# ZhendongWang6/Uformer

Hardware: AMD Instinct MI355X
Metric: restored images/sec (256x256, Uformer-B) (higher is better)
Workload: dtype bf16

## Files before the change

### include/uformer_hip.h

```cpp
#ifndef UFORMER_HIP_H
#define UFORMER_HIP_H

#include <stddef.h>
#include <stdint.h>

#ifdef __cplusplus
extern "C" {
#endif

#define UF_ABI_VERSION 1

typedef enum { UF_F32 = 0, UF_BF16 = 1, UF_F16 = 2 } uf_dtype;

#define UF_OK 0
#define UF_ERR_SHAPE (-1)
#define UF_ERR_UNSUPPORTED (-2)
#define UF_ERR_ALIGN (-3)
#define UF_ERR_LAUNCH (-4)
#define UF_ERR_WORKSPACE (-5)
#define UF_ERR_NULL (-6)

int uf_version(void);
int uf_last_error(char* buf, size_t n);

// ... 36 lines not shown

int uf_window_attention_fwd(const void* q, const void* k, const void* vt, const float* bias_dense,
                            const float* mask, int n_mask, void* out, int n_windows, int heads,
                            int head_dim, int H, int W, int shift, uf_dtype dtype, void* stream);

int uf_dwconv3x3_gelu_fwd(const void* x, const float* w9, const float* bias, void* out, int B,
                          int H, int W, int C, uf_dtype dtype, void* stream);
int uf_dwconv3x3_fwd(const void* x, const float* w9, const float* bias, void* out, int B, int H,
                     int W, int C, int gelu, uf_dtype dtype, void* stream);

int uf_dwconv3x3_pre_gelu_fwd(const void* x, const float* w9, const float* bias, void* pre_out, void* act_out, int B, int H,
                              int W, int C, uf_dtype dtype, void* stream);
int uf_dwconv3x3_gelu_in_pre_gelu_fwd(const void* pre_in, const float* w9, const float* bias, void* pre_out, void* act_out, int B, int H,
                                      int W, int C, uf_dtype dtype, void* stream);
int uf_dwconv3x3_mul_dgelu(const void* dy, const float* w9_flipped, const void* pre, void* out, int B, int H, int W, int C,
                           uf_dtype dtype, void* stream);

int uf_dwconv_linear2_fwd(const void* h1, const float* w9, const float* bdw, const void* W2_fm,
                          const float* b2, float* x, int ld, int B, int H, int W, int C,
                          uf_dtype dtype, void* stream);

typedef struct uf_block_params {
    const float* norm1_w;
    const float* norm1_b;
    const float* modulator;
    const float* rpb_dense;
    const float* rpb_fm;
    const float* rpb_tab;
    const void* wqkv_fm;
    const float* bqkv;
    const void* wproj;
    const void* wproj_fm;
    const float* bproj;
    const float* norm2_w;
    const float* norm2_b;
    const void* w1_fm;
    const float* b1;
    const float* wdw9;
    const float* bdw;
    const void* w2_fm;
    const float* b2;
    int32_t shift;
    int32_t heads;
    const float* qkv_dw9;
    const float* qkv_bdw;
} uf_block_params;

size_t uf_block_workspace_bytes(int M, int C, uf_dtype dtype);

int uf_lewin_attn_fwd(const uf_block_params* p, float* x, int ld, int B, int H, int W, int C,
                      const float* user_mask, int n_mask, uf_dtype dtype, void* ws,
                      size_t ws_bytes, void* stream);
int uf_leff_fwd(const uf_block_params* p, float* x, int ld, int B, int H, int W, int C,
                uf_dtype dtype, void* ws, size_t ws_bytes, void* stream);
int uf_ffn_fwd(float* x, int ld, const float* gamma, const float* beta, const void* W1_fm, const float* b1, const void* W2_fm,
               const float* b2, const float* scale, int B, int M, int C, uf_dtype dtype, void* stream);
int uf_mlp_fwd(const uf_block_params* p, float* x, int ld, int B, int H, int W, int C, uf_dtype dtype, void* ws, size_t ws_bytes,
               void* stream);
int uf_lewin_attn_train_fwd(const uf_block_params* p, const float* x, int ld, float* x1, int ld1, int B, int H, int W, int C,
                            const float* drop_attn, uf_dtype dtype, void* xn, void* q, void* k, void* vt, void* o, void* z, void* a1,
                            void* stream);
int uf_lewin_block_fwd(const uf_block_params* p, float* x, int ld, int B, int H, int W, int C,
                       const float* user_mask, int n_mask, uf_dtype dtype, void* ws,
                       size_t ws_bytes, void* stream);

int uf_lewin_block_train_fwd(const uf_block_params* p, float* x, int ld, int B, int H, int W, int C,
                             const float* drop_attn, const float* drop_leff, uf_dtype dtype, void* ws,
                             size_t ws_bytes, void* stream);

int uf_downsample_fwd(const float* x, int ld_x, const void* w, const float* bias, float* out,
                      int ld_o, int B, int H, int W, int C, uf_dtype dtype, void* stream);
int uf_downsample_fm_fwd(const float* x, int ld_x, const void* w, const void* w_fm, const float* bias, float* out,
                         int ld_o, int B, int H, int W, int C, uf_dtype dtype, void* stream);
int uf_upsample_fwd(const float* x, int ld_x, const void* w, const float* bias, float* out,
                    int ld_o, int B, int H, int W, int Cin, int Cout, uf_dtype dtype, void* stream);
int uf_input_proj_fwd(const float* img, const float* w27, const float* bias, float* out, int ld_o,
                      int B, int Cin, int H, int W, int E, void* stream);
int uf_output_proj_fwd(const float* x, int ld_x, const float* w, const float* bias,
                       const float* img, float* out, int B, int H, int W, int C2, int add_img,
                       void* stream);
int uf_output_proj_c_fwd(const float* x, int ld_x, const float* w, const float* bias,
                         const float* img, float* out, int B, int H, int W, int C2, int Cout, int add_img,
                         void* stream);

int uf_gelu_bwd(const void* a, const void* dy, void* dx, long long n, uf_dtype dtype, void* stream);
int uf_gelu_fwd(const void* a, void* y, long long n, uf_dtype dtype, void* stream);
int uf_linear_pre_gelu_fwd(const void* A, const void* W, const float* bias, void* out, void* act_out, int M, int N, int K,
                           uf_dtype dtype, void* stream);
int uf_linear_mul_dgelu(const void* A, const void* W, const float* bias, const void* pre, void* out, int M, int N, int K,
                        uf_dtype dtype, void* stream);
int uf_linear_residual_fwd(const void* A, const void* W, const float* bias, const float* resid, float* out, const float* scale,
                           int B, int H, int Wd, int N, int K, int windowed, int shift, uf_dtype dtype, void* stream);
size_t uf_layernorm_bwd_workspace_bytes(int rows, int C);
int uf_layernorm_bwd(const float* x, int ld_x, const float* gamma, const float* dy, int ld_dy, float* dx, int ld_dx,
                     float* dgamma, float* dbeta, int rows, int C, void* ws, size_t ws_bytes, void* stream);
int uf_layernorm_bwd_fused(const float* x, int ld_x, const float* gamma, const void* dy, int ld_dy, int dy_is_f32,
                           const float* add, float* dx, int ld_dx, float* dgamma, float* dbeta, int B, int H, int W, int C,
                           int windowed, int shift, uf_dtype dtype, void* ws, size_t ws_bytes, void* stream);
int uf_layernorm_bwd_cast(const float* x, int ld_x, const float* gamma, const void* dy, int ld_dy, int dy_is_f32,
                          const float* add, float* dx, int ld_dx, float* dgamma, float* dbeta, int B, int H, int W, int C,
                          int windowed, int shift, uf_dtype dtype, void* cast_out, const float* cast_scale, int cast_windowed, int cast_shift,
                          void* ws, size_t ws_bytes, void* stream);
size_t uf_linear_wgrad_workspace_bytes(int M, int N, int K);
int uf_linear_wgrad(const void* dY, int ldy, const void* X, int ldx, float* dW, float* db, int M, int N, int K,
                    uf_dtype dtype, void* ws, size_t ws_bytes, void* stream);
size_t uf_window_attention_bwd_workspace_bytes(int n_windows, int heads);
int uf_window_attention_bwd(const void* q, const void* k, const void* vt, const float* bias_dense, const float* mask,
                            int n_mask, const void* dO, int ldo, void* dq, void* dk, void* dvt, float* dbias,
                            int n_windows, int heads, int head_dim, int H, int W, int shift, uf_dtype dtype,
                            void* ws, size_t ws_bytes, void* stream);
int uf_window_attention_bwd_qkv(const void* q, const void* k, const void* vt, const float* bias_dense, const float* mask,
                                int n_mask, const void* dO, int ldo, void* dqkv, float* dbias, int n_windows, int heads,
                                int head_dim, int H, int W, int shift, uf_dtype dtype, void* ws, size_t ws_bytes, void* stream);
size_t uf_dwconv3x3_wgrad_workspace_bytes(int C, uf_dtype dtype);
int uf_dwconv3x3_wgrad(const void* h, const void* dc, float* dw9, float* dbias, int B, int H, int W, int C,
                       uf_dtype dtype, void* ws, size_t ws_bytes, void* stream);
size_t uf_dwconv3x3_bwd_workspace_bytes(int C, uf_dtype dtype);
int uf_dwconv3x3_bwd(const void* dc, const float* w9_flipped, const void* pre, void* da, float* dw9, float* dbias,
                     int B, int H, int W, int C, uf_dtype dtype, void* ws, size_t ws_bytes, void* stream);

size_t uf_rows_sum_workspace_bytes(int M, int N);
int uf_rows_sum(const void* X, int ld, float* out, int M, int N, uf_dtype dtype, void* ws, size_t ws_bytes, void* stream);
int uf_rpb_table_grad(const float* dbias_dense, float* dtable, int heads, void* stream);
int uf_im2col(const float* x, int ld_x, void* cols, int ldc, int B, int H, int W, int Cin, int k, int stride, int pad,
              int nchw, uf_dtype dtype, void* stream);
int uf_col2im(const void* dcols, int ldc, float* dx, int ld_dx, int B, int H, int W, int Cin, int k, int stride, int pad,
              int nchw, int accumulate, uf_dtype dtype, void* stream);

size_t uf_conv3x3_bwd_workspace_bytes(int B, int H, int W, int Cin, int Cout);
int uf_conv3x3_bwd(const float* x, int x_nchw, const float* dy, const float* act_out, float slope, const float* w, float* dx,
                   float* dW, float* db, int B, int H, int W, int Cin, int Cout, void* ws, size_t ws_bytes, void* stream);

int uf_residual_combine(const float* a, const void* b, int b_is_f32, float* out, const float* scale, int B, int H, int W,
                        int C, int windowed, int shift, uf_dtype dtype, void* stream);
int uf_grad_fork(const float* g1, const float* g2, float* sum_out, void* cast_out, const float* scale, int B, int H, int W,
                 int C, int windowed, int shift, uf_dtype dtype, void* stream);
int uf_qkv_grad_merge(const void* dq, const void* dk, const void* dvt, void* dqkv, int n_windows, int heads, int head_dim,
                      uf_dtype dtype, void* stream);

typedef struct uf_block_train_params {
    const float* norm1_w;  const float* norm1_b;  const float* norm2_w;  const float* norm2_b;
    const float* modulator;
    const float* rpb_dense;
    const void* wqkv;
    const void* wqkv_t;
    const float* bqkv;
    const void* wproj;  const void* wproj_t;  const float* bproj;
    const void* w1;     const void* w1_t;     const float* b1;
    const float* wdw9;  const float* wdw9_flip;  const float* bdw;
    const void* w2_t;
    int32_t shift, heads;
    const void* w2;
} uf_block_train_params;
typedef struct uf_block_grads {
    float* norm1_w;  float* norm1_b;  float* norm2_w;  float* norm2_b;
    float* modulator;
    float* rpb_table;
    float* wqkv;  float* bqkv;
    float* wproj; float* bproj;
    float* w1;    float* b1;
    float* wdw;   float* bdw;
    float* w2;    float* b2;
} uf_block_grads;
typedef struct uf_block_raw_params {
    const float* norm1_w;  const float* norm1_b;  const float* norm2_w;  const float* norm2_b;
    const float* modulator;
// ... 146 lines not shown
```

### uformer_amd/_lib.py

```python
from __future__ import annotations

import ctypes as C
import os
import threading

_HERE = os.path.dirname(os.path.abspath(__file__))
LIB_PATH = os.path.join(_HERE, "lib", "libuformer_hip.so")
LIB_PATH = os.environ.get("UFORMER_HIP_LIB", LIB_PATH)

UF_F32, UF_BF16, UF_F16 = 0, 1, 2

c_int, c_void_p, c_size_t, c_float_p = C.c_int, C.c_void_p, C.c_size_t, C.c_void_p


class BlockParams(C.Structure):
    _fields_ = [(n, C.c_void_p) for n in (
        "norm1_w", "norm1_b", "modulator", "rpb_dense", "rpb_fm", "rpb_tab", "wqkv_fm", "bqkv", "wproj", "wproj_fm", "bproj",
        "norm2_w", "norm2_b", "w1_fm", "b1", "wdw9", "bdw", "w2_fm", "b2")] + [
        ("shift", C.c_int32), ("heads", C.c_int32), ("qkv_dw9", C.c_void_p), ("qkv_bdw", C.c_void_p)]


class BlockTrainParams(C.Structure):
    _fields_ = [(n, C.c_void_p) for n in (
        "norm1_w", "norm1_b", "norm2_w", "norm2_b", "modulator", "rpb_dense", "wqkv", "wqkv_t", "bqkv", "wproj", "wproj_t", "bproj",
# ... 24 lines not shown
class ModelDesc(C.Structure):
    _fields_ = [
        ("embed_dim", C.c_int32), ("dd_in", C.c_int32), ("in_chans", C.c_int32),
        ("depths", C.c_int32 * 9),
        ("blocks", C.POINTER(BlockParams)),
        ("in_w27", C.c_void_p), ("in_b", C.c_void_p), ("out_w", C.c_void_p), ("out_b", C.c_void_p),
        ("down_w", C.c_void_p * 4), ("down_b", C.c_void_p * 4),
        ("up_w", C.c_void_p * 4), ("up_b", C.c_void_p * 4),
        ("down_w_fm", C.c_void_p * 4),
        ("cross", C.POINTER(CrossParams)),
    ]


class UnetDesc(C.Structure):
    _fields_ = [
        ("dim", C.c_int32),
        ("in_w27", C.c_void_p), ("in_b", C.c_void_p), ("c11_w1", C.c_void_p), ("c11_b1", C.c_void_p),
        ("w0", C.c_void_p * 9), ("b0", C.c_void_p * 9), ("w2", C.c_void_p * 9), ("b2", C.c_void_p * 9),
        ("w11", C.c_void_p * 9), ("b11", C.c_void_p * 9),
        ("pool_w", C.c_void_p * 4), ("pool_b", C.c_void_p * 4), ("up_w", C.c_void_p * 4), ("up_b", C.c_void_p * 4),
        ("out_w", C.c_void_p), ("out_b", C.c_void_p),
    ]


P = c_void_p
I = c_int
SIGNATURES = {
    "uf_version": (I, []),
    "uf_last_error": (I, [C.c_char_p, c_size_t]),
    "uf_timing_enable": (I, [I]),
    "uf_timing_report": (I, [C.c_char_p, c_size_t]),
    "uf_debug_set_tbuf": (I, [P]),
    "uf_weight_fm_elems": (c_size_t, [I, I]),
    "uf_pack_weight_fm": (I, [P, P, I, I, I, P]),
    "uf_window_partition": (I, [P, P, I, I, I, I, I, I, P]),
    "uf_window_reverse": (I, [P, P, I, I, I, I, I, I, P]),
    "uf_shift_mask": (I, [P, I, I, I, P]),
    "uf_layernorm_fwd": (I, [P, I, P, P, P, P, I, I, I, I, I, I, I, P]),
    "uf_linear_fwd": (I, [P, P, P, P, I, I, I, I, I, P]),
    "uf_qkv_fwd": (I, [P, P, P, P, P, P, I, I, I, I, P]),
    "uf_ln_qkv_fwd": (I, [P, I, P, P, P, P, P, P, P, P, I, I, I, I, I, I, I, P]),
    "uf_ln_convqkv_fwd": (I, [P, I, P, P, P, P, P, P, P, P, P, P, I, I, I, I, I, I, I, P]),
    "uf_ln_linear_gelu_fwd": (I, [P, I, P, P, P, P, P, I, I, I, I, P]),
    "uf_window_attention_fwd": (I, [P, P, P, P, P, I, P, I, I, I, I, I, I, I, P]),
    "uf_dwconv3x3_gelu_fwd": (I, [P, P, P, P, I, I, I, I, I, P]),
    "uf_dwconv3x3_fwd": (I, [P, P, P, P, I, I, I, I, I, I, P]),
    "uf_gelu_bwd": (I, [P, P, P, C.c_longlong, I, P]),
    "uf_gelu_fwd": (I, [P, P, C.c_longlong, I, P]),
    "uf_linear_pre_gelu_fwd": (I, [P, P, P, P, P, I, I, I, I, P]),
    "uf_linear_mul_dgelu": (I, [P, P, P, P, P, I, I, I, I, P]),
    "uf_dwconv3x3_pre_gelu_fwd": (I, [P, P, P, P, P, I, I, I, I, I, P]),
    "uf_dwconv3x3_gelu_in_pre_gelu_fwd": (I, [P, P, P, P, P, I, I, I, I, I, P]),
    "uf_dwconv3x3_mul_dgelu": (I, [P, P, P, P, I, I, I, I, I, P]),
    "uf_linear_residual_fwd": (I, [P, P, P, P, P, P, I, I, I, I, I, I, I, I, P]),
    "uf_layernorm_bwd_workspace_bytes": (c_size_t, [I, I]),
    "uf_layernorm_bwd": (I, [P, I, P, P, I, P, I, P, P, I, I, P, c_size_t, P]),
    "uf_layernorm_bwd_fused": (I, [P, I, P, P, I, I, P, P, I, P, P, I, I, I, I, I, I, I, P, c_size_t, P]),
    "uf_layernorm_bwd_cast": (I, [P, I, P, P, I, I, P, P, I, P, P, I, I, I, I, I, I, I, P, P, I, I, P, c_size_t, P]),
    "uf_linear_wgrad_workspace_bytes": (c_size_t, [I, I, I]),
    "uf_linear_wgrad": (I, [P, I, P, I, P, P, I, I, I, I, P, c_size_t, P]),
    "uf_window_attention_bwd_workspace_bytes": (c_size_t, [I, I]),
    "uf_window_attention_bwd": (I, [P, P, P, P, P, I, P, I, P, P, P, P, I, I, I, I, I, I, I, P, c_size_t, P]),
    "uf_window_attention_bwd_qkv": (I, [P, P, P, P, P, I, P, I, P, P, I, I, I, I, I, I, I, P, c_size_t, P]),
    "uf_dwconv3x3_wgrad_workspace_bytes": (c_size_t, [I, I]),
    "uf_dwconv3x3_wgrad": (I, [P, P, P, P, I, I, I, I, I, P, c_size_t, P]),
    "uf_dwconv3x3_bwd_workspace_bytes": (c_size_t, [I, I]),
    "uf_dwconv3x3_bwd": (I, [P, P, P, P, P, P, I, I, I, I, I, P, c_size_t, P]),
    "uf_dwconv_linear2_fwd": (I, [P, P, P, P, P, P, I, I, I, I, I, I, P]),
    "uf_block_workspace_bytes": (c_size_t, [I, I, I]),
    "uf_lewin_attn_fwd": (I, [C.POINTER(BlockParams), P, I, I, I, I, I, P, I, I, P, c_size_t, P]),
    "uf_leff_fwd": (I, [C.POINTER(BlockParams), P, I, I, I, I, I, I, P, c_size_t, P]),
    "uf_ffn_fwd": (I, [P, I, P, P, P, P, P, P, P, I, I, I, I, P]),
    "uf_cross_attn_fwd": (I, [C.POINTER(CrossParams), P, I, I, I, I, P]),
    "uf_mlp_fwd": (I, [C.POINTER(BlockParams), P, I, I, I, I, I, I, P, c_size_t, P]),
    "uf_lewin_attn_train_fwd": (I, [C.POINTER(BlockParams), P, I, P, I, I, I, I, I, P, I, P, P, P, P, P, P, P, P]),
    "uf_lewin_block_fwd": (I, [C.POINTER(BlockParams), P, I, I, I, I, I, P, I, I, P, c_size_t, P]),
    "uf_lewin_block_train_fwd": (I, [C.POINTER(BlockParams), P, I, I, I, I, I, P, P, I, P, c_size_t, P]),
    "uf_downsample_fwd": (I, [P, I, P, P, P, I, I, I, I, I, I, P]),
    "uf_downsample_fm_fwd": (I, [P, I, P, P, P, P, I, I, I, I, I, I, P]),
    "uf_upsample_fwd": (I, [P, I, P, P, P, I, I, I, I, I, I, I, P]),
    "uf_input_proj_fwd": (I, [P, P, P, P, I, I, I, I, I, I, P]),
    "uf_output_proj_fwd": (I, [P, I, P, P, P, P, I, I, I, I, I, P]),
    "uf_output_proj_c_fwd": (I, [P, I, P, P, P, P, I, I, I, I, I, I, P]),
    "uf_rows_sum_workspace_bytes": (c_size_t, [I, I]),
    "uf_rows_sum": (I, [P, I, P, I, I, I, P, c_size_t, P]),
    "uf_rpb_table_grad": (I, [P, P, I, P]),
    "uf_im2col": (I, [P, I, P, I, I, I, I, I, I, I, I, I, I, P]),
    "uf_col2im": (I, [P, I, P, I, I, I, I, I, I, I, I, I, I, I, P]),
    "uf_pack_block_train_bytes": (C.c_size_t, [I, I, I]),
    "uf_pack_block_train": (I, [P, I, I, I, I, P, C.c_size_t, P, P, P]),
    "uf_lewin_block_bwd_workspace_bytes": (C.c_size_t, [I, I, I, I, I, I]),
    "uf_lewin_block_bwd": (I, [P, P, P, P, P, P, P, I, I, I, I, I, P, C.c_size_t, P]),
    "uf_leff_bwd": (I, [P, P, P, P, P, P, I, I, I, I, I, P, C.c_size_t, P]),
    "uf_lewin_attn_bwd": (I, [P, P, P, P, P, P, I, I, I, I, I, P, C.c_size_t, P]),
    "uf_downsample_bwd_workspace_bytes": (C.c_size_t, [I, I, I, I, I, I]),
    "uf_downsample_bwd": (I, [P, I, P, P, P, I, I, P, P, I, I, I, I, I, I, P, C.c_size_t, P]),
    "uf_upsample_cat_bwd_workspace_bytes": (C.c_size_t, [I, I, I, I, I, I]),
    "uf_upsample_cat_bwd": (I, [P, I, P, I, P, P, P, P, I, I, I, I, I, I, P, C.c_size_t, P]),
    "uf_conv3x3_bwd_workspace_bytes": (C.c_size_t, [I, I, I, I, I]),
    "uf_conv3x3_bwd": (I, [P, I, P, P, C.c_float, P, P, P, P, I, I, I, I, I, P, C.c_size_t, P]),
    "uf_residual_combine": (I, [P, P, I, P, P, I, I, I, I, I, I, I, P]),
    "uf_grad_fork": (I, [P, P, P, P, P, I, I, I, I, I, I, I, P]),
    "uf_qkv_grad_merge": (I, [P, P, P, P, I, I, I, I, P]),
    "uf_charbonnier_workspace_bytes": (c_size_t, [C.c_longlong]),
    "uf_charbonnier_fwd_bwd": (I, [P, P, P, P, C.c_longlong, C.c_float, C.c_float, P, c_size_t, P]),
    "uf_adamw_step": (I, [P, P, P, P, P, I, C.c_double, C.c_double, C.c_double, C.c_double, C.c_double, I, C.c_double, P]),
    "uf_grad_scaler_check": (I, [P, P, I, P, P]),
    "uf_adamw_step_scaled": (I, [P, P, P, P, P, I, C.c_double, C.c_double, C.c_double, C.c_double, C.c_double, C.c_double, P, P]),
    "uf_grad_scaler_update": (I, [P, C.c_double, C.c_double, I, P]),
    "uf_image_metric_workspace_bytes": (c_size_t, [I, I, I, I]),
    "uf_batch_mse": (I, [P, P, P, I, I, I, I, I, P, c_size_t, P]),
    "uf_batch_ssim": (I, [P, P, P, I, I, I, I, P, c_size_t, P]),
    "uf_expand2square": (I, [P, P, P, I, I, I, I, I, P]),
    "uf_crop_clamp": (I, [P, P, I, I, I, I, I, I, P]),
    "uf_expand_canvas": (I, [P, P, P, I, I, I, I, I, I, P]),
    "uf_crop_clamp_canvas": (I, [P, P, I, I, I, I, I, I, I, P]),
    "uf_crop_augment": (I, [P, I, I, P, P, I, I, I, I, I, P]),
    "uf_crop_augment_c": (I, [P, I, I, P, P, I, I, I, I, I, I, P]),
    "uf_mixup": (I, [P, P, P, P, I, C.c_longlong, P]),
    "uf_uformer_workspace_bytes": (c_size_t, [C.POINTER(ModelDesc), I, I, I, I]),
    "uf_uformer_fwd": (I, [C.POINTER(ModelDesc), P, P, I, I, I, I, P, c_size_t, P]),
    "uf_window4_attention_fwd": (I, [P, I, P, P, I, I, I, I, I, I, I, P]),
    "uf_window4_attention_bwd": (I, [P, I, P, P, I, P, I, P, I, I, I, I, I, I, P]),
    "uf_rpb4_table_grad": (I, [P, P, I, I, P]),
    "uf_window4_partition": (I, [P, P, I, I, I, I, I, P]),
    "uf_window4_reverse": (I, [P, P, I, I, I, I, I, P]),
    "uf_lewin_block4_fwd": (I, [C.POINTER(Block4Params), P, I, I, I, I, I, P, P, I, P, c_size_t, P]),
    "uf_uformer_win4_workspace_bytes": (c_size_t, [C.POINTER(ModelDesc), I, I, I, I]),
    "uf_uformer_win4_fwd": (I, [C.POINTER(ModelDesc), C.POINTER(Block4Params), P, P, I, I, I, I, P, c_size_t, P]),
    "uf_conv_packed_elems": (c_size_t, [I, I, I]),
    "uf_conv3x3_fwd": (I, [P, I, P, P, P, I, P, I, I, I, I, I, I, I, I, I, P]),
    "uf_conv1x1_fwd": (I, [P, I, P, P, P, I, I, I, I, I, I, I, P]),
    "uf_conv4s2_fwd": (I, [P, I, P, P, P, I, I, I, I, I, I, I, P]),
    "uf_conv1x1_nchw_fwd": (I, [P, P, P, P, I, I, I, I, I, I, P]),
    "uf_unet_workspace_bytes": (c_size_t, [C.POINTER(UnetDesc), I, I, I, I]),
    "uf_unet_fwd": (I, [C.POINTER(UnetDesc), P, P, I, I, I, I, P, c_size_t, P]),
}

_lock = threading.Lock()
_lib = None


class UformerHipError(RuntimeError):
    pass


def load():
    global _lib
    if _lib is not None:
        return _lib
    with _lock:
        if _lib is not None:
            return _lib
        if not os.path.exists(LIB_PATH):
            raise UformerHipError(
                f"{LIB_PATH} not found: build it with `python __graft_entry__.py` "
                "(hipcc --offload-arch=gfx950).  There is no CPU / PyTorch fallback for the hot path.")
        lib = C.CDLL(LIB_PATH)
        older = os.environ.get("UF_ALLOW_OLDER_LIB") == "1"
        for name, (res, args) in SIGNATURES.items():
            if older and not hasattr(lib, name):
                continue
            fn = getattr(lib, name)
            fn.restype = res
            fn.argtypes = args
        if lib.uf_version() != 1:
# ... 15 lines not shown
```

### uformer_amd/csrc/uf_elementwise.hip

```cpp
#include "uf_internal.h"

namespace uf {
namespace {

template <bool REVERSE>
__global__ void window_copy_kernel(const u32x4* __restrict__ src, u32x4* __restrict__ dst, int rows, int chunks_per_row,
                                   int H, int W, int shift) {
    const long long idx = (long long)blockIdx.x * blockDim.x + threadIdx.x;
    if (idx >= (long long)rows * chunks_per_row) return;
    const int m = (int)(idx / chunks_per_row), c = (int)(idx - (long long)m * chunks_per_row);
    const int tok = window_row_to_token(m, H, W, shift);
    if (REVERSE) dst[(size_t)tok * chunks_per_row + c] = src[(size_t)m * chunks_per_row + c];
    else dst[(size_t)m * chunks_per_row + c] = src[(size_t)tok * chunks_per_row + c];
}

template <bool REVERSE, typename E>
__global__ void window_copy_elem_kernel(const E* __restrict__ src, E* __restrict__ dst, int rows, int C, int H, int W, int shift) {
    const long long idx = (long long)blockIdx.x * blockDim.x + threadIdx.x;
    if (idx >= (long long)rows * C) return;
    const int m = (int)(idx / C), c = (int)(idx - (long long)m * C);
    const int tok = window_row_to_token(m, H, W, shift);
    if (REVERSE) dst[(size_t)tok * C + c] = src[(size_t)m * C + c];
    else dst[(size_t)m * C + c] = src[(size_t)tok * C + c];
}

template <typename T, int C>
__global__ __launch_bounds__(256) void layernorm_kernel(const float* __restrict__ x, int ld_x, const float* __restrict__ gamma,
                                                        const float* __restrict__ beta, const float* __restrict__ modulator,
                                                        T* __restrict__ out, int rows, int H, int W, int windowed, int shift) {
    constexpr int LPR = (C / 4) < 64 ? (C / 4) : 64;
    constexpr int V4 = C / (4 * LPR);
    constexpr int RPB = 256 / LPR;
    const int sub = threadIdx.x % LPR;
    const int m = blockIdx.x * RPB + threadIdx.x / LPR;
    const bool live = m < rows;
    const int mc = live ? m : rows - 1;
    const int src = windowed ? window_row_to_token(mc, H, W, shift) : mc;
    f32x4 v[V4];
    float sum = 0.f;
#pragma unroll
    for (int i = 0; i < V4; ++i) {
        v[i] = *reinterpret_cast<const f32x4*>(x + (size_t)src * ld_x + (i * LPR + sub) * 4);
        sum += (v[i][0] + v[i][1]) + (v[i][2] + v[i][3]);
    }
    sum = allreduce<RedSum, LPR>(sum);
    const float mean = sum * (1.0f / C);
    float sq = 0.f;
#pragma unroll
    for (int i = 0; i < V4; ++i) {
        v[i] -= mean;
        sq += (v[i][0] * v[i][0] + v[i][1] * v[i][1]) + (v[i][2] * v[i][2] + v[i][3] * v[i][3]);
    }
    sq = allreduce<RedSum, LPR>(sq);
    const float rstd = 1.0f / sqrtf(sq * (1.0f / C) + 1e-5f);
    if (!live) return;
#pragma unroll
    for (int i = 0; i < V4; ++i) {
        const int c = (i * LPR + sub) * 4;
        const f32x4 g = *reinterpret_cast<const f32x4*>(gamma + c);
        const f32x4 b = *reinterpret_cast<const f32x4*>(beta + c);
        f32x4 y = v[i] * rstd * g + b;
        if (modulator) y += *reinterpret_cast<const f32x4*>(modulator + (size_t)(m & 63) * C + c);
        store4(out + (size_t)m * C + c, y);
    }
}

template <typename T> struct Vec16 {
    static_assert(sizeof(T) == 2, "2-byte operand type");
    static constexpr int N = 8;
    static __device__ __forceinline__ void load(const T* p, float* f) { unpack8<T>(*reinterpret_cast<const u32x4*>(p), f); }
    static __device__ __forceinline__ void store(T* p, const float* f) { *reinterpret_cast<u32x4*>(p) = pack8<T>(f); }
};
template <> struct Vec16<float> {
    static constexpr int N = 4;
    static __device__ __forceinline__ void load(const float* p, float* f) {
        const f32x4 r = *reinterpret_cast<const f32x4*>(p);
        f[0] = r[0]; f[1] = r[1]; f[2] = r[2]; f[3] = r[3];
    }
    static __device__ __forceinline__ void store(float* p, const float* f) {
        *reinterpret_cast<f32x4*>(p) = f32x4{f[0], f[1], f[2], f[3]};
    }
};

// ... 664 lines not shown
        }
#undef UF_IP2
        return check_launch("input_proj");
    }
    if (px == 8) hipLaunchKernelGGL(input_proj_kernel<8>, dim3((nx + 255) / 256, H, B), dim3(256), 0, (hipStream_t)stream, img, w27, bias, out, ld_o, B, Cin, H, W, E);
    else hipLaunchKernelGGL(input_proj_kernel<4>, dim3((nx + 255) / 256, H, B), dim3(256), 0, (hipStream_t)stream, img, w27, bias, out, ld_o, B, Cin, H, W, E);
    return check_launch("input_proj");
}

extern "C" int uf_output_proj_c_fwd(const float* x, int ld_x, const float* w, const float* bias, const float* img, float* out,
                                    int B, int H, int W, int C2, int Cout, int add_img, void* stream) {
    UF_REQUIRE(x && w && bias && out && (!add_img || img), UF_ERR_NULL, "uf_output_proj_fwd: null pointer");
    UF_REQUIRE(B > 0 && H > 0 && W > 0 && ld_x >= C2 && ld_x % 4 == 0, UF_ERR_SHAPE, "uf_output_proj_fwd: bad shape");
    UF_REQUIRE(Cout >= 1 && Cout <= 4, UF_ERR_UNSUPPORTED, "uf_output_proj_fwd: Cout=%d unsupported (1..4)", Cout);
    UF_REQUIRE((long long)B * H * W * ld_x < 0xffffffffLL && H / OP_R < 65535 && B <= 65535, UF_ERR_SHAPE, "uf_output_proj_fwd: tensor too large for 32-bit indexing");
    hipStream_t st = (hipStream_t)stream;
    const long long pix = (long long)B * H * W;
    ScopedTimer tm("output_proj", 18.0 * Cout * pix * C2, 4.0 * pix * (C2 + 2 * Cout), st);
#define UF_OP_CO(LAUNCH)                                                    \
    switch (Cout) {                                                         \
        case 1: LAUNCH(1) break;                                            \
        case 2: LAUNCH(2) break;                                            \
        case 3: LAUNCH(3) break;                                            \
        default: LAUNCH(4) break;                                           \
    }
    {
        const bool v1 = variant("head", 2) == 1;
        if (!v1 && (C2 == 16 || C2 == 32 || C2 == 64) && (long long)B * H * W * ld_x * 4 < 0xffffff00LL) {
            const int lpp = C2 / 4, tw = 2 * (256 / lpp), tiles_x = (W + tw - 1) / tw, tiles_y = (H + OP_R - 1) / OP_R;
            const int smem = (6 * (tw + 2) * C2 * 4 + 1023) / 1024 * 1024;
            const long long nt = (long long)tiles_x * tiles_y * B;
            if (nt < 0x7fffffffLL) {
#define UF_OP2(LPPV, COV)                                                                                                                             \
                {                                                                                                                                     \
                    auto kern = output_proj2_kernel<LPPV, COV>;                                                                                       \
                    static bool lds_done[64] = {};                                                                                                    \
                    if (int rc = ensure_dynamic_lds(reinterpret_cast<const void*>(kern), smem, lds_done, "output_proj")) return rc;                  \
                    hipLaunchKernelGGL(kern, dim3((unsigned)nt), dim3(256), smem, st, x, ld_x, w, bias, img, out, B, H, W, add_img, tiles_x, tiles_y); \
                }
#define UF_OP2_4(COV) UF_OP2(4, COV)
#define UF_OP2_8(COV) UF_OP2(8, COV)
#define UF_OP2_16(COV) UF_OP2(16, COV)
                if (lpp == 4) { UF_OP_CO(UF_OP2_4) } else if (lpp == 8) { UF_OP_CO(UF_OP2_8) } else { UF_OP_CO(UF_OP2_16) }
#undef UF_OP2_4
#undef UF_OP2_8
#undef UF_OP2_16
#undef UF_OP2
                return check_launch("output_proj");
            }
        }
    }
#define UF_OP1(LPPV, COV)                                                                                                               \
    {                                                                                                                                   \
        const unsigned nx = (unsigned)W * LPPV;                                                                                         \
        hipLaunchKernelGGL((output_proj_kernel<LPPV, COV>), dim3((nx + 255) / 256, (H + OP_R - 1) / OP_R, B), dim3(256), 0, st, x, ld_x, \
                           w, bias, img, out, B, H, W, add_img);                                                                        \
    }
#define UF_OP1_4(COV) UF_OP1(4, COV)
#define UF_OP1_8(COV) UF_OP1(8, COV)
#define UF_OP1_16(COV) UF_OP1(16, COV)
#define UF_OP1_32(COV) UF_OP1(32, COV)
    switch (C2) {
        case 16: UF_OP_CO(UF_OP1_4) break;
        case 32: UF_OP_CO(UF_OP1_8) break;
        case 64: UF_OP_CO(UF_OP1_16) break;
        case 128: UF_OP_CO(UF_OP1_32) break;
        default:
            set_error("uf_output_proj_fwd: C2=%d unsupported (16,32,64,128)", C2);
            return UF_ERR_UNSUPPORTED;
    }
#undef UF_OP1_4
#undef UF_OP1_8
#undef UF_OP1_16
#undef UF_OP1_32
#undef UF_OP1
#undef UF_OP_CO
    return check_launch("output_proj");
}

extern "C" int uf_output_proj_fwd(const float* x, int ld_x, const float* w, const float* bias, const float* img, float* out,
                                  int B, int H, int W, int C2, int add_img, void* stream) {
    return uf_output_proj_c_fwd(x, ld_x, w, bias, img, out, B, H, W, C2, 3, add_img, stream);
}
```

### uformer_amd/csrc/uf_internal.h

```cpp
#pragma once
#include "uf_common.h"

namespace uf {

enum ALoad { A_PLAIN = 0, A_FROM_R = 1, A_CONV_DOWN = 2 };
enum Epi {
    E_STORE_T = 0,
    E_STORE_T_GELU = 1,
    E_QKV = 2,
    E_RES_WINREV = 3,
    E_RES = 4,
    E_STORE_R = 5,
    E_UPSAMPLE = 6,
    E_STORE_T_PRE_GELU = 7,
    E_STORE_T_MUL_DGELU = 8
};

struct GemmParams {
    const void* A; int lda;
    const void* W;
    const void* W_fm = nullptr;
    const float* bias;
    int M, N, K;
    int H, W_, C;
    int shift;
    void* out; int ldo;
    const float* resid; int ldr;
    void* q; void* k; void* vt; int heads, hd; float qscale;
    int Cout;
    void* aux;
    const float* scale; int hw;
};

int launch_gemm(const GemmParams& p, int aload, int epi, uf_dtype dtype, hipStream_t stream);
int launch_down_dx(const void* dyT, int ld_dy, const void* w_pk_t, void* wc, float* dx, int ld_dx, int B, int H, int W, int Cin, int Cout, int accumulate, uf_dtype dtype,
                   hipStream_t st, bool* done);

constexpr int MAX_SIDE = 7, MAX_LANE_EVENTS = 8;
struct Lane { hipStream_t s[MAX_SIDE] = {}; hipEvent_t fork = nullptr, join[MAX_SIDE] = {}; int n = 0; hipEvent_t ev[MAX_LANE_EVENTS] = {}; int n_ev = 0; };
Lane* acquire_lane(int want, int* dev_out);
void release_lane(Lane* ln, int dev);
bool lane_events(Lane* ln, int want);

void debug_set_tbuf(void* p);
bool attn_block_supported(const uf_block_params* bp, const float* user_mask, uf_dtype dtype, int C, int heads);
int launch_attn_block(const uf_block_params* bp, float* x, int ld, int B, int H, int W, int C, uf_dtype dtype, void* h1_out, hipStream_t st,
                      const float* drop = nullptr, float* xo = nullptr, int ldo = 0);
int launch_leff2(const void* h1, const float* w9, const float* bdw, const void* W2, const float* b2, float* x, int ld, int B, int H, int W, int C,
                 uf_dtype dtype, const float* drop, hipStream_t st);

int launch_attn_block_train(const uf_block_params* bp, const float* x, int ld, float* x1, int ld1, int B, int H, int W, int C, uf_dtype dtype, const float* drop,
                            void* xn, void* q, void* k, void* vt, void* o, void* z, void* a1, hipStream_t st);

}
```

### uformer_amd/csrc/uf_leff2.hip

```cpp
#include <stdlib.h>

#include "uf_internal.h"
#include "uf_mconv.h"

namespace uf {
namespace {

struct Leff2Params {
    const void* h1;
    const float* w9; const float* bdw;
    const void* W2; const float* b2;
    float* x; int ld;
    const float* drop;
    int B, H, W;
    int n_tiles;
    unsigned long long* tbuf;
};

constexpr int KCW = 64;

template <typename T> __device__ __forceinline__ void cvt8(const char* p, float* f);
template <> __device__ __forceinline__ void cvt8<bf16>(const char* p, float* f) { unpack8<bf16>(*reinterpret_cast<const u32x4*>(p), f); }
template <> __device__ __forceinline__ void cvt8<f16>(const char* p, float* f) { unpack8<f16>(*reinterpret_cast<const u32x4*>(p), f); }
template <> __device__ __forceinline__ void cvt8<float>(const char* p, float* f) {
    const f32x4 a = *reinterpret_cast<const f32x4*>(p), b = *reinterpret_cast<const f32x4*>(p + 16);
    f[0] = a[0]; f[1] = a[1]; f[2] = a[2]; f[3] = a[3]; f[4] = b[0]; f[5] = b[1]; f[6] = b[2]; f[7] = b[3];
}
__device__ __forceinline__ void put8(bf16* p, const float* f) { *reinterpret_cast<u32x4*>(p) = pack8<bf16>(f); }
__device__ __forceinline__ void put8(f16* p, const float* f) { *reinterpret_cast<u32x4*>(p) = pack8<f16>(f); }
__device__ __forceinline__ void put8(float* p, const float* f) {
    *reinterpret_cast<f32x4*>(p) = f32x4{f[0], f[1], f[2], f[3]};
    *reinterpret_cast<f32x4*>(p + 4) = f32x4{f[4], f[5], f[6], f[7]};
}

template <typename T, int C, int NPG, int NC, int NBUF, int WPS, int PW = 4, int CP = 0>
__global__ __launch_bounds__((PW * NPG + NC) * 64, WPS) void leff2_kernel(const Leff2Params p) {
    constexpr int NP = PW * NPG;
    constexpr int MC = sizeof(T) == 2 ? 1 : 0;
    static_assert(PW == 4 || (PW == 8 && MC != 0), "8 producer waves per group: MFMA stencil only (two pixel tiles per wave)");
    static_assert(CP == 0 || (MC != 0 && PW == 4 && NPG == 1 && NC == 4 * CP), "consumer stencil jobs: MFMA stencil, 4 producers, one job per consumer wave");
    constexpr int PTW = 16 / PW - CP;
    constexpr int SR = 2;
    constexpr int SZ = sizeof(T);
    constexpr int TH = 8, TW = 8, BM = 64;
    constexpr int HID = 4 * C;
    constexpr int KC = KCW * NPG;
    constexpr int NIT = HID / KC;
    static_assert(HID % KC == 0, "interval width");
    constexpr int HW_ = TW + 2, HT = (TH + 2) * HW_;
    constexpr int PS = KCW * SZ;
    constexpr int CPP = PS / 16;
    constexpr int HGB = (HT * PS + 1023) / 1024 * 1024;
    constexpr int NHG = HGB / 1024;
    constexpr int TRB = KC * 4;
    constexpr int TGB = (10 * TRB + 1023) / 1024 * 1024;
    constexpr int NTI = TGB / 1024;
    constexpr int NHI = NPG * NHG;
    constexpr int NI = NHI + NTI;
    constexpr int NS = (NI + NP - 1) / NP;
    constexpr int BUFB = NPG * HGB + TGB;
    constexpr int SAT = KC * SZ + 16;
    constexpr int AT_BYTES = BM * SAT;
    constexpr int WN = (C / 16) < NC ? (C / 16) : NC, WM = NC / WN;
    static_assert(WM <= 4, "consumer grid");
    constexpr int TMW = 4 / WM, TNW = (C / 16) / WN;
    extern __shared__ __attribute__((aligned(16))) char smem[];
    char* Ring = smem;
    char* At0 = smem + NBUF * BUFB;

    const int tid = threadIdx.x, lane = tid & 63;
    const int wave = __builtin_amdgcn_readfirstlane(tid >> 6);
    const bool producer = wave < NP;
    const int fr = lane & 15, fg = lane >> 4;
    const int tiles_x = p.W / TW, tiles_y = p.H / TH;
    const int G = (int)gridDim.x;
    const int nk = (p.n_tiles - (int)blockIdx.x + G - 1) / G;
    const int NTOT = nk * NIT;
    const int bt = xcd_tile(blockIdx.x, p.n_tiles);
    auto tile_coords = [&](int k, int& b, int& y0, int& x0) {
        const int t = xcd_tile((int)blockIdx.x + k * G, p.n_tiles);
        b = t / (tiles_x * tiles_y);
        const int tr = t - b * (tiles_x * tiles_y);
        y0 = (tr / tiles_x) * TH; x0 = (tr % tiles_x) * TW;
    };
    const T* W2 = reinterpret_cast<const T*>(p.W2);

    const unsigned hshift = (fr & 1) * 16;
    unsigned msk[4];
#pragma unroll
    for (int d = 0; d < 4; ++d) msk[d] = ((fg & 1) == (fr >> 3) && d == ((fr & 7) >> 1)) ? 0xffffffffu : 0u;
    const int gq = (producer ? wave : wave - NP) & 3;
    int boff[5];
#pragma unroll
    for (int ks = 0; ks < 5; ++ks) {
        int tap = 2 * ks + (fg >> 1);
        tap = tap < 9 ? tap : 8;
        const int hy = (fr >> 3) + tap / 3, hx = (fr & 7) + tap % 3;
        boff[ks] = ((hy * HW_ + hx) * 8 + ((gq * 2 + (fg & 1)) ^ (hx & 6))) * 16;
    }
    Census census; census.begin();
    if (producer) {
        const unsigned lds0 = (unsigned)(uintptr_t)(__attribute__((address_space(3))) char*)smem;
        const unsigned lds_dummy = lds0 + NBUF * BUFB + 2 * AT_BYTES;
        u32x4 rsrc = {0u, 0u, (unsigned)__builtin_amdgcn_readfirstlane((int)((unsigned)(p.H * p.W) * (unsigned)(HID * SZ))), 0x00020000u};
        unsigned voff[NS];
        int issue_k = -1;
        auto set_issue_tile = [&](int k) {
            int b, y0, x0;
            tile_coords(k, b, y0, x0);
            const unsigned long long ia = (unsigned long long)(uintptr_t)(reinterpret_cast<const char*>(p.h1) + (size_t)b * p.H * p.W * HID * SZ);
            rsrc[0] = (unsigned)__builtin_amdgcn_readfirstlane((int)(unsigned)ia);
            rsrc[1] = (unsigned)__builtin_amdgcn_readfirstlane((int)(unsigned)(ia >> 32)) & 0xffffu;
#pragma unroll
            for (int s = 0; s < NS; ++s) {
                const int idx = wave + s * NP;
                voff[s] = 0xffffff00u;
                if (idx < NHI) {
                    const int g = idx / NHG, q = (idx - g * NHG) * 64 + lane;
                    const int hp = q / CPP, part = q - hp * CPP;
                    const int hy = hp / HW_, hx = hp - hy * HW_;
                    const int iy = y0 + hy - 1, ix = x0 + hx - 1;
                    const int piece = MC ? (part ^ (hx & 6)) : part;
                    if (hp < HT && iy >= 0 && iy < p.H && ix >= 0 && ix < p.W) voff[s] = ((unsigned)(iy * p.W + ix) * (unsigned)HID + (unsigned)(g * KCW)) * (unsigned)SZ + (unsigned)(piece * 16);
                }
            }
            issue_k = k;
        };
        auto issue = [&](int m) {
            const int k = m / NIT, it = m - k * NIT;
            if (k != issue_k) set_issue_tile(k);
            const unsigned slot = lds0 + (unsigned)(m % NBUF) * BUFB;
#pragma unroll
            for (int s = 0; s < NS; ++s) {
                const int idx = wave + s * NP;
                if (idx < NHI) {
                    dma_buffer_to_lds(rsrc, voff[s], (unsigned)(it * KC * SZ), slot + (unsigned)idx * 1024u);
                } else if (idx < NI) {
                    const int q = (idx - NHI) * 64 + lane;
                    int row = q / (KC / 4);
                    const int c4 = (q - row * (KC / 4)) * 4;
                    row = row > 9 ? 9 : row;
                    const float* src = (row < 9 ? p.w9 + (size_t)row * HID : p.bdw) + it * KC + c4;
                    dma_global_to_lds(src, slot + NPG * HGB + (unsigned)(idx - NHI) * 1024u);
                } else {
                    dma_buffer_to_lds(rsrc, 0xffffff00u, 0u, lds_dummy);
                }
            }
// ... 53 lines not shown
            t1 = __builtin_readcyclecounter(); tw += t1 - t0; t0 = t1;
            if (NBUF >= 3 && i + NBUF - 1 < NTOT) wait_dma<(NBUF - 2) * NS>(); else wait_dma<0>();
            lds_barrier();
            t1 = __builtin_readcyclecounter(); tbar += t1 - t0; t0 = t1;
        }
        if (p.tbuf && lane == 0 && (bt & 63) == 0) { p.tbuf[((bt >> 6) * 16 + wave) * 4] = tw; p.tbuf[((bt >> 6) * 16 + wave) * 4 + 1] = tbar; p.tbuf[((bt >> 6) * 16 + wave) * 4 + 2] = producer; }
        return;
    }

    const int cw = wave - NP;
    const int wm = cw / WN, wn = cw % WN;
    constexpr int WKS = (SZ == 4 && TNW >= 4) ? 1 : 2;
    Frag<T> wf[WKS][TNW];
    const __amdgpu_buffer_rsrc_t wrs = __builtin_amdgcn_make_buffer_rsrc(const_cast<T*>(W2), 0, C * HID * SZ, 0x00020000);
    const int wlane = lane * 8 * SZ;
    auto w2_load = [&](int sub, int ks, int slot) {
#pragma unroll
        for (int i = 0; i < TNW; ++i) {
            const int soff = (((wn * TNW + i) * (HID / 32) + sub * 2 + ks) * 64) * 8 * SZ;
            if constexpr (SZ == 2) {
                wf[slot][i].v = __builtin_bit_cast(u32x4, __builtin_amdgcn_raw_buffer_load_b128(wrs, wlane, soff, 0));
            } else {
                wf[slot][i].lo = __builtin_bit_cast(f32x4, __builtin_amdgcn_raw_buffer_load_b128(wrs, wlane, soff, 0));
                wf[slot][i].hi = __builtin_bit_cast(f32x4, __builtin_amdgcn_raw_buffer_load_b128(wrs, wlane + 16, soff, 0));
            }
        }
    };
    auto w2_issue = [&](int sub) {
        if constexpr (WKS == 2) { w2_load(sub, 0, 0); w2_load(sub, 1, 1); }
    };

    f32x4 acc[TNW][TMW];
#pragma unroll
    for (int i = 0; i < TNW; ++i)
#pragma unroll
        for (int j = 0; j < TMW; ++j) acc[i][j] = f32x4{0.f, 0.f, 0.f, 0.f};

    constexpr bool XPRE = SZ == 2 && TNW * TMW <= 4 && CP == 0;
    f32x4 xres[XPRE ? TNW : 1][XPRE ? TMW : 1];
    auto x_ptr = [&](int b, int y0, int x0, int i, int j) -> float* {
        const int n = (wn * TNW + i) * 16 + fg * 4;
        const int pm = (wm * TMW + j) * 16 + fr;
        return p.x + ((size_t)(b * p.H + y0 + (pm >> 3)) * p.W + x0 + (pm & 7)) * p.ld + n;
    };
    w2_issue(0);
    lds_barrier();
    unsigned long long ctw = 0, ctbar = 0, ct0 = __builtin_readcyclecounter(), ct1;
#pragma unroll 1
    for (int j = 0; j <= NTOT; ++j) {
        if (j >= 1) {
            const int m = j - 1, k = m / NIT, it = m - k * NIT;
            int tb = 0, ty0 = 0, tx0 = 0;
            if (it == NIT - 1) {
                tile_coords(k, tb, ty0, tx0);
                if constexpr (XPRE) {
#pragma unroll
                    for (int i = 0; i < TNW; ++i)
#pragma unroll
                        for (int jj = 0; jj < TMW; ++jj) xres[i][jj] = *reinterpret_cast<const f32x4*>(x_ptr(tb, ty0, tx0, i, jj));
                }
            }
            const char* At = At0 + (m & 1) * AT_BYTES;
#pragma unroll
            for (int g = 0; g < NPG; ++g) {
                const int sub = it * NPG + g;
#pragma unroll
                for (int ks = 0; ks < 2; ++ks) {
                    if constexpr (WKS == 1) w2_load(sub, ks, 0);
                    Frag<T> af[TMW];
#pragma unroll
                    for (int jj = 0; jj < TMW; ++jj)
                        load_frag(af[jj], reinterpret_cast<const T*>(At + ((wm * TMW + jj) * 16 + fr) * SAT + (g * KCW + ks * 32 + fg * 8) * SZ));
                    __builtin_amdgcn_sched_barrier(0);
#pragma unroll
                    for (int ii = 0; ii < TNW; ++ii)
#pragma unroll
                        for (int jj = 0; jj < TMW; ++jj) mma16(acc[ii][jj], wf[WKS == 2 ? ks : 0][ii], af[jj]);
                    __builtin_amdgcn_sched_barrier(0);
                }
                if (sub + 1 < NIT * NPG) w2_issue(sub + 1);
                else if (j < NTOT) w2_issue(0);
                __builtin_amdgcn_sched_barrier(0);
            }
            if (it == NIT - 1) {
                const float dscale = p.drop ? p.drop[tb] : 1.0f;
#pragma unroll
                for (int i = 0; i < TNW; ++i) {
                    const f32x4 b2 = *reinterpret_cast<const f32x4*>(p.b2 + (wn * TNW + i) * 16 + fg * 4);
#pragma unroll
                    for (int jj = 0; jj < TMW; ++jj) {
                        float* xp = x_ptr(tb, ty0, tx0, i, jj);
                        f32x4 r;
                        if constexpr (XPRE) r = xres[i][jj]; else r = *reinterpret_cast<const f32x4*>(xp);
                        *reinterpret_cast<f32x4*>(xp) = r + (acc[i][jj] + b2) * dscale;
                        acc[i][jj] = f32x4{0.f, 0.f, 0.f, 0.f};
                    }
                }
            }
        }
        if constexpr (CP > 0) {
            if (j < NTOT) {
                const char* Hs = Ring + (j % NBUF) * BUFB;
                const float* Wl = reinterpret_cast<const float*>(Ring + (j % NBUF) * BUFB + NPG * HGB);
                mconv_job<T, 1, KC, SAT, 2 * HW_ * PS>(Hs, Wl, At0 + (j & 1) * AT_BYTES, gq, 4 - CP + (cw >> 2), boff, msk, hshift, fr, fg);
            }
        }
        ct1 = __builtin_readcyclecounter(); ctw += ct1 - ct0; ct0 = ct1;
        lds_barrier();
        ct1 = __builtin_readcyclecounter(); ctbar += ct1 - ct0; ct0 = ct1;
    }
    if (p.tbuf && lane == 0 && (bt & 63) == 0) { p.tbuf[((bt >> 6) * 16 + wave) * 4] = ctw; p.tbuf[((bt >> 6) * 16 + wave) * 4 + 1] = ctbar; p.tbuf[((bt >> 6) * 16 + wave) * 4 + 2] = 0; }
    if (cw == 0 && lane == 0) {
        Census c2 = census;
        if (p.tbuf) { unsigned long long* o = p.tbuf + 65536 + (size_t)bt * 8; o[0] = c2.t0; o[1] = __builtin_readcyclecounter(); o[2] = c2.r0; o[3] = wall_clock64();
            o[4] = (unsigned long long)__builtin_amdgcn_s_getreg((31 << 11) | 4) | ((unsigned long long)__builtin_amdgcn_s_getreg((31 << 11) | 20) << 32); }
    }
}

template <typename T, int C, int NPG, int NC, int NBUF, int WPS, int PW = 4, int CP = 0>
int launch_v(const Leff2Params& p, hipStream_t st) {
    constexpr int SZ = sizeof(T), KC = KCW * NPG;
    constexpr int HGB = (100 * KCW * SZ + 1023) / 1024 * 1024, TGB = (10 * KC * 4 + 1023) / 1024 * 1024;
    constexpr int smem = NBUF * (NPG * HGB + TGB) + 2 * 64 * (KC * SZ + 16) + 1024;
    static_assert(smem <= 160 * 1024, "LDS budget");
    auto kern = leff2_kernel<T, C, NPG, NC, NBUF, WPS, PW, CP>;
    static bool lds_done[64] = {};
    if (int rc = ensure_dynamic_lds(reinterpret_cast<const void*>(kern), smem, lds_done, "leff2")) return rc;
    const long long M = (long long)p.B * p.H * p.W;
    char name[96] = "";
    if (timing_enabled()) snprintf(name, sizeof(name), "leff2_%s_c%d_np%d_nc%d %lldx%dx%d", TypeName<T>::s, C, PW * NPG, NC, M, C, 4 * C);
    {
        ScopedTimer tm(name, 2.0 * M * C * 4 * C + 18.0 * M * 4 * C, (double)M * 4 * C * SZ + (double)M * C * 8, st);
        const int pe = variant("persist", -1);
        const bool pays = C <= 32 || C >= 256 || (C == 128 && p.n_tiles <= 1024);
        const bool persist = pe >= 0 ? pe != 0 : pays;
        constexpr int waves = PW * NPG + NC;
        constexpr int by_lds = (160 * 1024) / smem, by_waves = 32 / waves, by_regs = (WPS * 4) / waves > 0 ? (WPS * 4) / waves : 1;
        constexpr int per_cu = by_lds < by_waves ? (by_lds < by_regs ? by_lds : by_regs) : (by_waves < by_regs ? by_waves : by_regs);
        const int resident = 256 * (per_cu < 1 ? 1 : per_cu);
        int grid = p.n_tiles;
        if (persist && p.n_tiles > resident) {
            const int rounds = (p.n_tiles + resident - 1) / resident;
            grid = ((p.n_tiles + rounds - 1) / rounds + 7) / 8 * 8;
        }
        hipLaunchKernelGGL(kern, dim3((unsigned)grid), dim3(waves * 64), smem, st, p);
    }
    return check_launch("leff2");
}

constexpr int NB512 = 3, NB256 = 3, NB256E = 3;
template <typename T, int C>
int launch_c(const Leff2Params& p, hipStream_t st) {
    const int tiles = p.B * (p.H / 8) * (p.W / 8);
    if constexpr (sizeof(T) == 2 && C >= 32) {
        const int ev = variant("leff2", 0);
        const bool force = ev == 1, never = ev == 2;
        if constexpr (C == 128) { if (!never && (force || tiles <= 1024)) return launch_v<T, C, 1, 4, 2, 6, 8>(p, st); }
        else if constexpr (C == 256) { if (!never && (force || tiles <= 256)) return launch_v<T, C, 1, 8, NB256E, 4, 8>(p, st); }
        else if constexpr (C == 512) { if (force) return launch_v<T, C, 1, 8, 4, 4, 8>(p, st); }
        else { if (force) return launch_v<T, C, 1, 4, 2, 6, 8>(p, st); }
    }
    if constexpr (sizeof(T) == 2) {
        if constexpr (C <= 128) return launch_v<T, C, 1, 4, 2, 6>(p, st);
        else if constexpr (C == 256) return launch_v<T, C, 1, 4, NB256, 4>(p, st);
        else return launch_v<T, C, 1, 8, NB512, 3>(p, st);
    } else {
        (void)tiles;
        if constexpr (C <= 256) return launch_v<T, C, 1, 4, 2, 2>(p, st);
        else return launch_v<T, C, 1, 4, 2, 2>(p, st);
    }
}

template <typename T>
int launch_t(const Leff2Params& p, int C, hipStream_t st) {
    switch (C) {
        case 16: return launch_c<T, 16>(p, st);
        case 32: return launch_c<T, 32>(p, st);
        case 64: return launch_c<T, 64>(p, st);
        case 128: return launch_c<T, 128>(p, st);
        case 256: return launch_c<T, 256>(p, st);
        case 512: return launch_c<T, 512>(p, st);
        default:
            set_error("leff2: C=%d unsupported (16,32,64,128,256,512)", C);
            return UF_ERR_UNSUPPORTED;
    }
}

}
unsigned long long* debug_get_tbuf();
}

using namespace uf;

namespace uf {
int launch_leff2(const void* h1, const float* w9, const float* bdw, const void* W2, const float* b2, float* x, int ld, int B, int H, int W, int C,
                 uf_dtype dtype, const float* drop, hipStream_t st) {
    UF_REQUIRE(h1 && w9 && bdw && W2 && b2 && x, UF_ERR_NULL, "uf_dwconv_linear2_fwd: null pointer");
    UF_REQUIRE(B > 0 && H >= 8 && W >= 8 && H % 8 == 0 && W % 8 == 0, UF_ERR_SHAPE, "uf_dwconv_linear2_fwd: B=%d H=%d W=%d (multiples of 8)", B, H, W);
    UF_REQUIRE(ld >= C && ld % 4 == 0, UF_ERR_ALIGN, "uf_dwconv_linear2_fwd: ld=%d", ld);
    UF_REQUIRE(((uintptr_t)h1 % 16) == 0 && ((uintptr_t)W2 % 16) == 0 && ((uintptr_t)x % 16) == 0 && ((uintptr_t)w9 % 16) == 0 &&
                   ((uintptr_t)bdw % 16) == 0 && ((uintptr_t)b2 % 16) == 0,
               UF_ERR_ALIGN, "uf_dwconv_linear2_fwd: operands must be 16-byte aligned");
    UF_REQUIRE((long long)H * W * 4LL * C * (long long)dtype_size(dtype) < 0xffffff00LL, UF_ERR_SHAPE,
               "uf_dwconv_linear2_fwd: one image of the hidden tensor must stay under 4 GiB (32-bit buffer offsets)");
    UF_REQUIRE((long long)B * H * W < 0x7fffffffLL / 4, UF_ERR_SHAPE, "uf_dwconv_linear2_fwd: too many tokens");
    Leff2Params p{};
    p.tbuf = debug_get_tbuf();
    p.h1 = h1; p.w9 = w9; p.bdw = bdw; p.W2 = W2; p.b2 = b2; p.x = x; p.ld = ld; p.B = B; p.H = H; p.W = W; p.drop = drop;
    p.n_tiles = B * (H / 8) * (W / 8);
    if (dtype == UF_BF16) return launch_t<bf16>(p, C, st);
    if (dtype == UF_F16) return launch_t<f16>(p, C, st);
    if (dtype == UF_F32) return launch_t<float>(p, C, st);
    set_error("uf_dwconv_linear2_fwd: dtype %d", (int)dtype);
    return UF_ERR_UNSUPPORTED;
}
}

extern "C" int uf_dwconv_linear2_fwd(const void* h1, const float* w9, const float* bdw, const void* W2, const float* b2,
                                     float* x, int ld, int B, int H, int W, int C, uf_dtype dtype, void* stream) {
    return uf::launch_leff2(h1, w9, bdw, W2, b2, x, ld, B, H, W, C, dtype, nullptr, (hipStream_t)stream);
}
```

### uformer_amd/csrc/uf_model.hip

```cpp
#include <stdlib.h>

#include <mutex>
#include <vector>

#include "uf_internal.h"

namespace uf {

int launch_layernorm(const float* x, int ld_x, const float* gamma, const float* beta, const float* modulator, void* out,
                     int rows, int H, int W, int C, int windowed, int shift, uf_dtype dtype, hipStream_t st);

int launch_unpack_weight_fm(const void* fm, void* w, int N, int K, uf_dtype dtype, hipStream_t st);

namespace {

struct BlockWs {
    char* a;
    char* h1;
    char* h2;
    char* wr;
};

bool wide_block(size_t C) { return C > 512; }

// ... 16 lines not shown
}

bool mlp_block(const uf_block_params* p) { return !p->wdw9 && !p->bdw; }

bool conv_block(const uf_block_params* p) { return p->qkv_dw9 && p->qkv_bdw; }

int check_block_args(const uf_block_params* p, const float* x, int ld, int B, int H, int W, int C, uf_dtype dtype) {
    UF_REQUIRE(p && x, UF_ERR_NULL, "block: null pointer");
    UF_REQUIRE(!p->qkv_dw9 == !p->qkv_bdw, UF_ERR_NULL, "block: qkv_dw9 and qkv_bdw must both be set (ConvProjection, token_projection = 'conv') or both be NULL");
    UF_REQUIRE(!(conv_block(p) && wide_block((size_t)C)), UF_ERR_UNSUPPORTED, "block: token_projection = 'conv' is built for C <= 512 (got C=%d)", C);
    UF_REQUIRE(!p->wdw9 == !p->bdw, UF_ERR_NULL, "block: wdw9 and bdw must both be set (LeFF) or both be NULL (Mlp, token_mlp = 'ffn')");
    UF_REQUIRE(!(mlp_block(p) && wide_block((size_t)C)), UF_ERR_UNSUPPORTED, "block: token_mlp = 'ffn' is built for C <= 512 (got C=%d)", C);
    UF_REQUIRE(dtype_ok(dtype), UF_ERR_UNSUPPORTED, "block: dtype %d", (int)dtype);
    UF_REQUIRE(B > 0 && H >= 8 && W >= 8 && H % 8 == 0 && W % 8 == 0, UF_ERR_SHAPE, "block: B=%d H=%d W=%d (H,W multiples of 8)", B, H, W);
    UF_REQUIRE(C >= 16 && C % 16 == 0 && ld >= C && ld % 4 == 0, UF_ERR_SHAPE, "block: C=%d ld=%d", C, ld);
    UF_REQUIRE(p->heads > 0 && C % p->heads == 0, UF_ERR_SHAPE, "block: C=%d heads=%d", C, p->heads);
    UF_REQUIRE(p->shift == 0 || p->shift == 4, UF_ERR_UNSUPPORTED, "block: shift=%d (0 or 4)", p->shift);
    UF_REQUIRE((long long)B * H * W * 4LL * C < 0x7fffffffLL * 4, UF_ERR_SHAPE, "block: tensor too large for 32-bit row indexing");
    return UF_OK;
}

int block_fwd(const uf_block_params* p, float* x, int ld, int B, int H, int W, int C, const float* user_mask, int n_mask, uf_dtype dtype,
              const BlockWs& w, hipStream_t st, const float* drop_attn, const float* drop_leff);

int attn_half(const uf_block_params* p, float* x, int ld, int B, int H, int W, int C, const float* user_mask, int n_mask,
              uf_dtype dtype, const BlockWs& w, hipStream_t st, bool* fc1_done = nullptr, const float* drop = nullptr) {
    const int M = B * H * W;
    const size_t sz = dtype_size(dtype);
    const int heads = p->heads, hd = C / heads;
    if (!conv_block(p) && attn_block_supported(p, user_mask, dtype, C, heads)) {
        const bool with_fc1 = fc1_done && dtype_half(dtype) && C >= 32 && !mlp_block(p);
        if (fc1_done) *fc1_done = with_fc1;
        return launch_attn_block(p, x, ld, B, H, W, C, dtype, with_fc1 ? w.h1 : nullptr, st, drop);
    }
    UF_REQUIRE(!drop, UF_ERR_UNSUPPORTED, "DropPath scales need the fused attention kernel (bf16 / f16, or f32 with C <= 256; no caller mask)");
    char* q = w.h1;
    char* k = q + (size_t)M * C * sz;
    char* vt = k + (size_t)M * C * sz;
    int rc;
    if (conv_block(p)) {
        rc = uf_ln_convqkv_fwd(x, ld, p->norm1_w, p->norm1_b, p->modulator, p->qkv_dw9, p->qkv_bdw, p->wqkv_fm, p->bqkv, q, k, vt, B, H, W, C, heads,
                               p->shift, dtype, st);
    } else if (wide_block(C)) {
        rc = launch_layernorm(x, ld, p->norm1_w, p->norm1_b, p->modulator, w.a, M, H, W, C, 1, p->shift, dtype, st);
        if (rc) return rc;
        rc = launch_unpack_weight_fm(p->wqkv_fm, w.wr, 3 * C, C, dtype, st);
        if (rc) return rc;
        rc = uf_qkv_fwd(w.a, w.wr, p->bqkv, q, k, vt, M, C, heads, dtype, st);
    } else {
        rc = uf_ln_qkv_fwd(x, ld, p->norm1_w, p->norm1_b, p->modulator, p->wqkv_fm, p->bqkv, q, k, vt, B, H, W, C, heads,
                           p->shift, dtype, st);
    }
    if (rc) return rc;
    rc = uf_window_attention_fwd(q, k, vt, p->rpb_dense, user_mask, n_mask, w.a, M / 64, heads, hd, H, W, p->shift, dtype, st);
    if (rc) return rc;
    GemmParams g{};
    g.A = w.a; g.lda = C; g.W = p->wproj; g.bias = p->bproj; g.M = M; g.N = C; g.K = C;
    g.H = H; g.W_ = W; g.shift = p->shift;
    g.out = x; g.ldo = ld; g.resid = x; g.ldr = ld;
    return launch_gemm(g, A_PLAIN, E_RES_WINREV, dtype, st);
}

bool ffn_prefers_unfused(uf_dtype dtype, int C) { return C == 512 && dtype_half(dtype); }

int mlp_half(const uf_block_params* p, float* x, int ld, int B, int H, int W, int C, uf_dtype dtype, const BlockWs& w, hipStream_t st,
             const float* drop) {
    const int M = B * H * W;
    UF_REQUIRE(p->norm2_w && p->norm2_b && p->w1_fm && p->b1 && p->w2_fm && p->b2, UF_ERR_NULL, "mlp: null parameter");
    UF_REQUIRE(!wide_block(C), UF_ERR_UNSUPPORTED, "mlp: token_mlp = 'ffn' is built for C <= 512 (got C=%d)", C);
    if ((variant("ffn", 0) == 1 || ffn_prefers_unfused(dtype, C)) && M >= C) {
        int rc = uf_ln_linear_gelu_fwd(x, ld, p->norm2_w, p->norm2_b, p->w1_fm, p->b1, w.h1, M, 4 * C, C, dtype, st);
        if (rc) return rc;
        rc = launch_unpack_weight_fm(p->w2_fm, w.h2, C, 4 * C, dtype, st);
        if (rc) return rc;
        GemmParams g{};
        g.A = w.h1; g.lda = 4 * C; g.W = w.h2; g.bias = p->b2; g.M = M; g.N = C; g.K = 4 * C;
        g.H = H; g.W_ = W; g.hw = H * W; g.scale = drop;
        g.out = x; g.ldo = ld; g.resid = x; g.ldr = ld;
        return launch_gemm(g, A_PLAIN, E_RES, dtype, st);
    }
    return uf_ffn_fwd(x, ld, p->norm2_w, p->norm2_b, p->w1_fm, p->b1, p->w2_fm, p->b2, drop, B, M, C, dtype, st);
}

int leff_half(const uf_block_params* p, float* x, int ld, int B, int H, int W, int C, uf_dtype dtype, const BlockWs& w,
              hipStream_t st, bool fc1_done = false, const float* drop = nullptr) {
    const int M = B * H * W;
    if (mlp_block(p)) return mlp_half(p, x, ld, B, H, W, C, dtype, w, st, drop);
    if (wide_block(C)) {
        UF_REQUIRE(!drop && !fc1_done, UF_ERR_UNSUPPORTED, "leff: C=%d runs unfused, without DropPath scales", C);
        int rc = launch_layernorm(x, ld, p->norm2_w, p->norm2_b, nullptr, w.a, M, H, W, C, 0, 0, dtype, st);
        if (rc) return rc;
        rc = launch_unpack_weight_fm(p->w1_fm, w.wr, 4 * C, C, dtype, st);
        if (rc) return rc;
        rc = uf_linear_fwd(w.a, w.wr, p->b1, w.h1, M, 4 * C, C, 1, dtype, st);
        if (rc) return rc;
        rc = uf_dwconv3x3_gelu_fwd(w.h1, p->wdw9, p->bdw, w.h2, B, H, W, 4 * C, dtype, st);
        if (rc) return rc;
        rc = launch_unpack_weight_fm(p->w2_fm, w.wr, C, 4 * C, dtype, st);
        if (rc) return rc;
        GemmParams g{};
        g.A = w.h2; g.lda = 4 * C; g.W = w.wr; g.bias = p->b2; g.M = M; g.N = C; g.K = 4 * C;
        g.H = H; g.W_ = W; g.hw = H * W;
        g.out = x; g.ldo = ld; g.resid = x; g.ldr = ld;
        return launch_gemm(g, A_PLAIN, E_RES, dtype, st);
    }
    if (!fc1_done) {
        int rc = uf_ln_linear_gelu_fwd(x, ld, p->norm2_w, p->norm2_b, p->w1_fm, p->b1, w.h1, M, 4 * C, C, dtype, st);
        if (rc) return rc;
    }
    return launch_leff2(w.h1, p->wdw9, p->bdw, p->w2_fm, p->b2, x, ld, B, H, W, C, dtype, drop, st);
}

int block_fwd(const uf_block_params* p, float* x, int ld, int B, int H, int W, int C, const float* user_mask, int n_mask, uf_dtype dtype,
              const BlockWs& w, hipStream_t st, const float* drop_attn, const float* drop_leff) {
    bool fc1_done = false;
    int rc = attn_half(p, x, ld, B, H, W, C, user_mask, n_mask, dtype, w, st, &fc1_done, drop_attn);
    if (rc) return rc;
    return leff_half(p, x, ld, B, H, W, C, dtype, w, st, fc1_done, drop_leff);
}

}
}

using namespace uf;

extern "C" size_t uf_block_workspace_bytes(int M, int C, uf_dtype dtype) {
    if (M <= 0 || C <= 0) return 0;
    return block_ws_bytes((size_t)M, (size_t)C, dtype);
}

extern "C" int uf_lewin_attn_fwd(const uf_block_params* p, float* x, int ld, int B, int H, int W, int C,
                                 const float* user_mask, int n_mask, uf_dtype dtype, void* ws, size_t ws_bytes, void* stream) {
    int rc = check_block_args(p, x, ld, B, H, W, C, dtype);
    if (rc) return rc;
    BlockWs w;
    rc = carve(w, ws, ws_bytes, (size_t)B * H * W, C, dtype);
    if (rc) return rc;
    return attn_half(p, x, ld, B, H, W, C, user_mask, n_mask, dtype, w, (hipStream_t)stream);
}

extern "C" int uf_leff_fwd(const uf_block_params* p, float* x, int ld, int B, int H, int W, int C, uf_dtype dtype, void* ws,
                           size_t ws_bytes, void* stream) {
    int rc = check_block_args(p, x, ld, B, H, W, C, dtype);
    if (rc) return rc;
    BlockWs w;
    rc = carve(w, ws, ws_bytes, (size_t)B * H * W, C, dtype);
    if (rc) return rc;
    return leff_half(p, x, ld, B, H, W, C, dtype, w, (hipStream_t)stream);
}

extern "C" int uf_mlp_fwd(const uf_block_params* p, float* x, int ld, int B, int H, int W, int C, uf_dtype dtype, void* ws,
                          size_t ws_bytes, void* stream) {
    int rc = check_block_args(p, x, ld, B, H, W, C, dtype);
    if (rc) return rc;
    UF_REQUIRE(mlp_block(p), UF_ERR_UNSUPPORTED, "uf_mlp_fwd: a LeFF block (wdw9 / bdw set): call uf_leff_fwd");
    BlockWs w;
    rc = carve(w, ws, ws_bytes, (size_t)B * H * W, C, dtype);
    if (rc) return rc;
    return mlp_half(p, x, ld, B, H, W, C, dtype, w, (hipStream_t)stream, nullptr);
}

extern "C" int uf_lewin_block_fwd(const uf_block_params* p, float* x, int ld, int B, int H, int W, int C,
                                  const float* user_mask, int n_mask, uf_dtype dtype, void* ws, size_t ws_bytes, void* stream) {
    int rc = check_block_args(p, x, ld, B, H, W, C, dtype);
    if (rc) return rc;
    BlockWs w;
    rc = carve(w, ws, ws_bytes, (size_t)B * H * W, C, dtype);
    if (rc) return rc;
    return block_fwd(p, x, ld, B, H, W, C, user_mask, n_mask, dtype, w, (hipStream_t)stream, nullptr, nullptr);
}

extern "C" int uf_lewin_attn_train_fwd(const uf_block_params* p, const float* x, int ld, float* x1, int ld1, int B, int H, int W, int C,
                                       const float* drop_attn, uf_dtype dtype, void* xn, void* q, void* k, void* vt, void* o, void* z, void* a1,
                                       void* stream) {
    int rc = check_block_args(p, x, ld, B, H, W, C, dtype);
    if (rc) return rc;
    UF_REQUIRE(!conv_block(p), UF_ERR_UNSUPPORTED, "uf_lewin_attn_train_fwd: token_projection = 'conv' runs inference only");
    UF_REQUIRE(x1 && xn && q && k && vt && o && z && a1, UF_ERR_NULL, "uf_lewin_attn_train_fwd: null output pointer");
    UF_REQUIRE(x1 != x && ld1 >= C && ld1 % 4 == 0, UF_ERR_SHAPE, "uf_lewin_attn_train_fwd: x1 must be out of place, ld1=%d", ld1);
    UF_REQUIRE(dtype_half(dtype) && attn_block_supported(p, nullptr, dtype, C, p->heads), UF_ERR_UNSUPPORTED,
               "uf_lewin_attn_train_fwd: bf16 / f16 operands, head_dim 32, C = 32 ... 512 and the compact bias table (got dtype %d, C=%d, heads=%d)", (int)dtype, C, p->heads);
    const uintptr_t al = (uintptr_t)x1 | (uintptr_t)xn | (uintptr_t)q | (uintptr_t)k | (uintptr_t)vt | (uintptr_t)o | (uintptr_t)z | (uintptr_t)a1;
    UF_REQUIRE((al % 16) == 0, UF_ERR_ALIGN, "uf_lewin_attn_train_fwd: outputs must be 16-byte aligned");
    return launch_attn_block_train(p, x, ld, x1, ld1, B, H, W, C, dtype, drop_attn, xn, q, k, vt, o, z, a1, (hipStream_t)stream);
}

extern "C" int uf_lewin_block_train_fwd(const uf_block_params* p, float* x, int ld, int B, int H, int W, int C, const float* drop_attn,
                                        const float* drop_leff, uf_dtype dtype, void* ws, size_t ws_bytes, void* stream) {
    int rc = check_block_args(p, x, ld, B, H, W, C, dtype);
    if (rc) return rc;
    UF_REQUIRE(!conv_block(p), UF_ERR_UNSUPPORTED, "uf_lewin_block_train_fwd: token_projection = 'conv' runs inference only");
    BlockWs w;
    rc = carve(w, ws, ws_bytes, (size_t)B * H * W, C, dtype);
    if (rc) return rc;
    return block_fwd(p, x, ld, B, H, W, C, nullptr, 0, dtype, w, (hipStream_t)stream, drop_attn, drop_leff);
}

extern "C" int uf_downsample_fwd(const float* x, int ld_x, const void* w, const float* bias, float* out, int ld_o, int B,
                                 int H, int W, int C, uf_dtype dtype, void* stream) {
    UF_REQUIRE(x && w && bias && out, UF_ERR_NULL, "uf_downsample_fwd: null pointer");
    UF_REQUIRE(B > 0 && H % 2 == 0 && W % 2 == 0 && H > 0 && W > 0, UF_ERR_SHAPE, "uf_downsample_fwd: H=%d W=%d", H, W);
    UF_REQUIRE(ld_x >= C && ld_o >= 2 * C && ld_o % 4 == 0, UF_ERR_SHAPE, "uf_downsample_fwd: ld_x=%d ld_o=%d C=%d", ld_x, ld_o, C);
    GemmParams g{};
    g.A = x; g.lda = ld_x; g.W = w; g.bias = bias; g.M = B * (H / 2) * (W / 2); g.N = 2 * C; g.K = 16 * C;
    g.H = H; g.W_ = W; g.C = C; g.out = out; g.ldo = ld_o;
    return launch_gemm(g, A_CONV_DOWN, E_STORE_R, dtype, (hipStream_t)stream);
}

extern "C" int uf_downsample_fm_fwd(const float* x, int ld_x, const void* w, const void* w_fm, const float* bias, float* out, int ld_o, int B,
                                    int H, int W, int C, uf_dtype dtype, void* stream) {
    UF_REQUIRE(x && w && bias && out, UF_ERR_NULL, "uf_downsample_fm_fwd: null pointer");
    UF_REQUIRE(B > 0 && H % 2 == 0 && W % 2 == 0 && H > 0 && W > 0, UF_ERR_SHAPE, "uf_downsample_fm_fwd: H=%d W=%d", H, W);
    UF_REQUIRE(ld_x >= C && ld_o >= 2 * C && ld_o % 4 == 0, UF_ERR_SHAPE, "uf_downsample_fm_fwd: ld_x=%d ld_o=%d C=%d", ld_x, ld_o, C);
    UF_REQUIRE(!w_fm || ((uintptr_t)w_fm % 16) == 0, UF_ERR_ALIGN, "uf_downsample_fm_fwd: w_fm must be 16-byte aligned");
    GemmParams g{};
    g.A = x; g.lda = ld_x; g.W = w; g.W_fm = dtype_half(dtype) ? w_fm : nullptr; g.bias = bias; g.M = B * (H / 2) * (W / 2); g.N = 2 * C; g.K = 16 * C;
    g.H = H; g.W_ = W; g.C = C; g.out = out; g.ldo = ld_o;
    return launch_gemm(g, A_CONV_DOWN, E_STORE_R, dtype, (hipStream_t)stream);
}

extern "C" int uf_upsample_fwd(const float* x, int ld_x, const void* w, const float* bias, float* out, int ld_o, int B, int H,
                               int W, int Cin, int Cout, uf_dtype dtype, void* stream) {
    UF_REQUIRE(x && w && bias && out, UF_ERR_NULL, "uf_upsample_fwd: null pointer");
    UF_REQUIRE(B > 0 && H > 0 && W > 0 && Cout % 4 == 0, UF_ERR_SHAPE, "uf_upsample_fwd: bad shape");
    UF_REQUIRE(ld_x >= Cin && ld_o >= Cout && ld_o % 4 == 0, UF_ERR_SHAPE, "uf_upsample_fwd: ld_x=%d ld_o=%d", ld_x, ld_o);
    GemmParams g{};
    g.A = x; g.lda = ld_x; g.W = w; g.bias = bias; g.M = B * H * W; g.N = 4 * Cout; g.K = Cin;
    g.H = H; g.W_ = W; g.Cout = Cout; g.out = out; g.ldo = ld_o;
    return launch_gemm(g, A_FROM_R, E_UPSAMPLE, dtype, (hipStream_t)stream);
}

// ... 5 lines not shown
    size_t M[9];
    size_t off_D[4];
    size_t off_P;
    size_t off_blk;
    size_t blk_bytes;
    size_t total;
};

int make_plan(Plan& pl, const uf_model_desc* d, int B, int H, int W, uf_dtype dtype, int bwin = 8) {
    UF_REQUIRE(d, UF_ERR_NULL, "model desc is null");
    const int unit = 16 * bwin;
    UF_REQUIRE(H % unit == 0 && H > 0, UF_ERR_SHAPE, "H=%d must be a positive multiple of %d (4 downsamplings x window %d)", H, unit, bwin);
    UF_REQUIRE(W % unit == 0 && W > 0, UF_ERR_SHAPE, "W=%d must be a positive multiple of %d (4 downsamplings x window %d)", W, unit, bwin);
    UF_REQUIRE(B > 0, UF_ERR_SHAPE, "B=%d", B);
    UF_REQUIRE(d->embed_dim >= 16 && d->embed_dim % 16 == 0, UF_ERR_SHAPE, "embed_dim=%d must be a multiple of 16", d->embed_dim);
    const int e = d->embed_dim;
    const int mult[9] = {1, 2, 4, 8, 16, 16, 8, 4, 2};
    const int div[9] = {1, 2, 4, 8, 16, 8, 4, 2, 1};
    size_t blk = 0;
    for (int s = 0; s < 9; ++s) {
        pl.C[s] = e * mult[s];
        pl.res_h[s] = H / div[s];
        pl.res_w[s] = W / div[s];
        pl.M[s] = (size_t)B * pl.res_h[s] * pl.res_w[s];
        const size_t b = block_ws_bytes(pl.M[s], pl.C[s], dtype);
        if (b > blk) blk = b;
    }
    size_t off = 0;
    for (int k = 0; k < 4; ++k) {
        pl.off_D[k] = off;
        off += align_up(pl.M[5 + k] * pl.C[5 + k] * sizeof(float), 256);
    }
    pl.off_P = off;
    off += align_up(pl.M[4] * pl.C[4] * sizeof(float), 256);
    pl.off_blk = off;
    pl.blk_bytes = blk;
    pl.total = off + blk;
    return UF_OK;
}
}

constexpr size_t WS_SPLIT_SLACK = 256 * 256;

static size_t ws_split_wide_extra(const uf_model_desc* d, uf_dtype dtype) {
    const size_t C = (size_t)16 * d->embed_dim;
    return wide_block(C) ? (size_t)MAX_SIDE * align_up(4 * C * C * dtype_size(dtype), 256) : 0;
}

extern "C" size_t uf_uformer_workspace_bytes(const uf_model_desc* d, int B, int H, int W, uf_dtype dtype) {
    Plan pl;
    if (make_plan(pl, d, B, H, W, dtype) != UF_OK) return 0;
    return pl.total + WS_SPLIT_SLACK + ws_split_wide_extra(d, dtype);
}

namespace {
int check_image_chans(const uf_model_desc* d) {
    UF_REQUIRE(d->dd_in >= 1 && d->dd_in <= 8, UF_ERR_UNSUPPORTED, "uf_uformer_fwd: dd_in=%d (1..8 supported)", d->dd_in);
    UF_REQUIRE(d->in_chans >= 1 && d->in_chans <= 4, UF_ERR_UNSUPPORTED, "uf_uformer_fwd: in_chans=%d (1..4 supported)", d->in_chans);
    UF_REQUIRE(d->dd_in != 3 || d->in_chans == 3, UF_ERR_UNSUPPORTED, "uf_uformer_fwd: dd_in=3 adds the input to the output (global residual), so in_chans=%d must be 3",
               d->in_chans);
    return UF_OK;
}
int forward_one_stream(const uf_model_desc* d, const uf_block4_params* bneck, const float* img, float* out, int B, int H, int W, uf_dtype dtype,
                       void* ws, size_t ws_bytes, void* stream) {
    Plan pl;
    int rc = make_plan(pl, d, B, H, W, dtype, bneck ? 4 : 8);
    if (rc) return rc;
    UF_REQUIRE(img && out && ws && d->blocks, UF_ERR_NULL, "uf_uformer_fwd: null pointer");
    UF_REQUIRE(((uintptr_t)ws % 256) == 0, UF_ERR_ALIGN, "uf_uformer_fwd: workspace must be 256-byte aligned");
    UF_REQUIRE(ws_bytes >= pl.total, UF_ERR_WORKSPACE, "uf_uformer_fwd: workspace too small: %zu < %zu", ws_bytes, pl.total);
    if (int rc2 = check_image_chans(d)) return rc2;
    hipStream_t st = (hipStream_t)stream;
    char* base = (char*)ws;
    float* D[4];
    for (int k = 0; k < 4; ++k) D[k] = (float*)(base + pl.off_D[k]);
    float* P = (float*)(base + pl.off_P);
    void* bws = base + pl.off_blk;

    auto enc_view = [&](int s, float*& ptr, int& ld) {
        ptr = D[3 - s] + pl.C[s];
        ld = 2 * pl.C[s];
    };
    const uf_block_params* blk = d->blocks;
    auto run_stage = [&](int s, float* x, int ld) -> int {
        for (int i = 0; i < d->depths[s]; ++i, ++blk) {
            const uf_cross_params* cr = (d->cross && !bneck) ? d->cross + (blk - d->blocks) : nullptr;
            if (cr && cr->wq_fm) {
                int r = uf_cross_attn_fwd(cr, x, ld, (int)pl.M[s], pl.C[s], dtype, st);
                if (r) return r;
            }
            int r =(s == 4 && bneck) ? uf_lewin_block4_fwd(bneck + i, x, ld, B, pl.res_h[s], pl.res_w[s], pl.C[s], nullptr, nullptr, dtype, bws, pl.blk_bytes, st)
                                      : uf_lewin_block_fwd(blk, x, ld, B, pl.res_h[s], pl.res_w[s], pl.C[s], nullptr, 0, dtype, bws, pl.blk_bytes, st);
            if (r) return r;
        }
        return UF_OK;
    };

    float* x; int ld;
    enc_view(0, x, ld);
    rc = uf_input_proj_fwd(img, d->in_w27, d->in_b, x, ld, B, d->dd_in, H, W, d->embed_dim, st);
    if (rc) return rc;
    for (int s = 0; s < 4; ++s) {
        rc = run_stage(s, x, ld);
        if (rc) return rc;
        float* nx; int nld;
        if (s < 3) enc_view(s + 1, nx, nld); else { nx = P; nld = pl.C[4]; }
        rc = uf_downsample_fm_fwd(x, ld, d->down_w[s], d->down_w_fm[s], d->down_b[s], nx, nld, B, pl.res_h[s], pl.res_w[s], pl.C[s], dtype, st);
        if (rc) return rc;
        x = nx; ld = nld;
    }
    rc = run_stage(4, x, ld);
    if (rc) return rc;
    for (int k = 0; k < 4; ++k) {
        const int s = 5 + k;
        const int cin = pl.C[s - 1], cout = pl.C[s] / 2;
        rc = uf_upsample_fwd(x, ld, d->up_w[k], d->up_b[k], D[k], pl.C[s], B, pl.res_h[s - 1], pl.res_w[s - 1], cin, cout, dtype, st);
        if (rc) return rc;
        x = D[k]; ld = pl.C[s];
        rc = run_stage(s, x, ld);
        if (rc) return rc;
    }
    return uf_output_proj_c_fwd(x, ld, d->out_w, d->out_b, img, out, B, H, W, pl.C[8], d->in_chans, d->dd_in == 3 ? 1 : 0, st);
}

}

namespace {
int forward_split(const uf_model_desc* d, const uf_block4_params* bneck, const float* img, float* out, int B, int H, int W, uf_dtype dtype,
                  void* ws, size_t ws_bytes, void* stream) {
    static const int env_streams = getenv("UF_STREAMS") ? atoi(getenv("UF_STREAMS")) : 0;
    int n = env_streams > 0 ? (env_streams > MAX_SIDE + 1 ? MAX_SIDE + 1 : env_streams) : (B >= 8 ? 2 : 1);
    if (n > B) n = B;
    if (n < 2 || timing_enabled()) return forward_one_stream(d, bneck, img, out, B, H, W, dtype, ws, ws_bytes, stream);
    UF_REQUIRE(d && img && out && ws, UF_ERR_NULL, "uf_uformer_fwd: null pointer");
    if (int rc = check_image_chans(d)) return rc;
    int dev = 0;
    Lane* ss = acquire_lane(n - 1, &dev);
    UF_REQUIRE(ss, UF_ERR_LAUNCH, "uf_uformer_fwd: could not create the side streams");
    struct LaneGuard { Lane* l; int d; ~LaneGuard() { release_lane(l, d); } } guard{ss, dev};
    hipStream_t st = (hipStream_t)stream;
    UF_REQUIRE(hipEventRecord(ss->fork, st) == hipSuccess, UF_ERR_LAUNCH, "uf_uformer_fwd: hipEventRecord failed");
    int rc_all = UF_OK, b0 = 0;
    size_t off = 0;
    for (int i = 0; i < n; ++i) {
        const int Bi = B / n + (i < B % n ? 1 : 0);
        Plan pl;
        int rc = make_plan(pl, d, Bi, H, W, dtype, bneck ? 4 : 8);
        if (rc) return rc;
        UF_REQUIRE(ws_bytes >= off + pl.total, UF_ERR_WORKSPACE, "uf_uformer_fwd: workspace too small for %d streams", n);
        hipStream_t si = i == 0 ? st : ss->s[i - 1];
        if (i > 0) hipStreamWaitEvent(si, ss->fork, 0);
        rc = forward_one_stream(d, bneck, img + (size_t)b0 * d->dd_in * H * W, out + (size_t)b0 * d->in_chans * H * W, Bi, H, W, dtype, (char*)ws + off,
                                pl.total, si);
        if (rc && !rc_all) rc_all = rc;
        if (i > 0) {
            hipEventRecord(ss->join[i - 1], si);
            hipStreamWaitEvent(st, ss->join[i - 1], 0);
        }
        off += align_up(pl.total, 256);
        b0 += Bi;
    }
    return rc_all;
}
}

extern "C" int uf_uformer_fwd(const uf_model_desc* d, const float* img, float* out, int B, int H, int W, uf_dtype dtype,
                              void* ws, size_t ws_bytes, void* stream) {
    return forward_split(d, nullptr, img, out, B, H, W, dtype, ws, ws_bytes, stream);
}

extern "C" size_t uf_uformer_win4_workspace_bytes(const uf_model_desc* d, int B, int H, int W, uf_dtype dtype) {
    Plan pl;
    if (make_plan(pl, d, B, H, W, dtype, 4) != UF_OK) return 0;
    return pl.total + WS_SPLIT_SLACK + ws_split_wide_extra(d, dtype);
}

extern "C" int uf_uformer_win4_fwd(const uf_model_desc* d, const uf_block4_params* bottleneck, const float* img, float* out, int B, int H, int W,
                                   uf_dtype dtype, void* ws, size_t ws_bytes, void* stream) {
    UF_REQUIRE(bottleneck, UF_ERR_NULL, "uf_uformer_win4_fwd: null bottleneck parameters");
    return forward_split(d, bottleneck, img, out, B, H, W, dtype, ws, ws_bytes, stream);
}
```

### uformer_amd/csrc/uf_pack.hip

```cpp
#include "uf_internal.h"

namespace uf {
namespace {

template <typename T> __device__ __forceinline__ void store8_t(T* p, const float* f) { *reinterpret_cast<u32x4*>(p) = pack8<T>(f); }
template <> __device__ __forceinline__ void store8_t<float>(float* p, const float* f) {
    *reinterpret_cast<f32x4*>(p) = f32x4{f[0], f[1], f[2], f[3]};
    *reinterpret_cast<f32x4*>(p + 4) = f32x4{f[4], f[5], f[6], f[7]};
}

struct MatJob { const float *src0, *src1; int n0, N, K; void *plain, *tr, *fm; };
template <typename T>
__device__ __forceinline__ void pack_linear_block(const MatJob& j, int blk) {
    const int kc = j.K / 8;
    const long long idx = (long long)blk * 256 + threadIdx.x;
    if (idx >= (long long)j.N * kc) return;
    const int n = (int)(idx / kc), k = (int)(idx % kc) * 8;
    const float* row = n < j.n0 ? j.src0 + (size_t)n * j.K : j.src1 + (size_t)(n - j.n0) * j.K;
    const f32x4 a = *reinterpret_cast<const f32x4*>(row + k), b = *reinterpret_cast<const f32x4*>(row + k + 4);
    const float f[8] = {a[0], a[1], a[2], a[3], b[0], b[1], b[2], b[3]};
    T *plain = (T*)j.plain, *tr = (T*)j.tr, *fm = (T*)j.fm;
    if (plain) store8_t<T>(plain + (size_t)n * j.K + k, f);
    if (fm) {
        const int KS = j.K / 32;
// ... 49 lines not shown
};

PackPlan plan_pack(int C, int heads, uf_dtype dtype) {
    const size_t sz = dtype_size(dtype), c2 = (size_t)C * C;
    size_t off = 0;
    auto take = [&](size_t bytes) { off = align_up(off, 256); const size_t o = off; off += bytes; return o; };
    PackPlan p;
    p.wqkv = take(3 * c2 * sz); p.wqkv_t = take(3 * c2 * sz); p.wqkv_fm = take(3 * c2 * sz);
    p.wp = take(c2 * sz);       p.wp_t = take(c2 * sz);       p.wp_fm = take(c2 * sz);
    p.w1 = take(4 * c2 * sz);   p.w1_t = take(4 * c2 * sz);   p.w1_fm = take(4 * c2 * sz);
    p.w2 = take(4 * c2 * sz);   p.w2_t = take(4 * c2 * sz);   p.w2_fm = take(4 * c2 * sz);
    p.bqkv = take((size_t)3 * C * 4); p.w9 = take((size_t)36 * C * 4); p.w9_flip = take((size_t)36 * C * 4);
    p.dense = take((size_t)heads * 4096 * 4); p.tab = take((size_t)heads * 225 * 4);
    p.total = align_up(off, 256);
    return p;
}

}
}

using namespace uf;

extern "C" size_t uf_pack_block_train_bytes(int C, int heads, uf_dtype dtype) {
    if (C <= 0 || heads <= 0 || !dtype_ok(dtype)) return 0;
    return plan_pack(C, heads, dtype).total;
}

extern "C" int uf_pack_block_train(const uf_block_raw_params* raw, int C, int heads, int shift, uf_dtype dtype, void* buf, size_t buf_bytes,
                                   uf_block_params* fwd, uf_block_train_params* bwd, void* stream) {
    UF_REQUIRE(raw && buf && (fwd || bwd), UF_ERR_NULL, "uf_pack_block_train: null pointer");
    UF_REQUIRE(dtype_ok(dtype), UF_ERR_UNSUPPORTED, "uf_pack_block_train: dtype %d", (int)dtype);
    UF_REQUIRE(C >= 32 && C % 32 == 0 && heads > 0 && C % heads == 0, UF_ERR_SHAPE, "uf_pack_block_train: C=%d heads=%d (C a multiple of 32)", C, heads);
    UF_REQUIRE(raw->norm1_w && raw->norm1_b && raw->norm2_w && raw->norm2_b && raw->rpb_table && raw->rpb_index && raw->to_q_w && raw->to_q_b && raw->to_kv_w &&
                   raw->to_kv_b && raw->proj_w && raw->proj_b && raw->lin1_w && raw->lin1_b && raw->dw_w && raw->dw_b && raw->lin2_w && raw->lin2_b,
               UF_ERR_NULL, "uf_pack_block_train: a parameter pointer is NULL (only modulator may be)");
    const PackPlan pl = plan_pack(C, heads, dtype);
    UF_REQUIRE(buf_bytes >= pl.total && ((uintptr_t)buf % 256) == 0, UF_ERR_WORKSPACE, "uf_pack_block_train: buffer %zu < %zu bytes (256-byte aligned)", buf_bytes, pl.total);
    hipStream_t st = (hipStream_t)stream;
    char* b = (char*)buf;
    auto at = [&](size_t o) { return (void*)(b + o); };
    SmallPack sp{raw->to_q_b, raw->to_kv_b, raw->dw_w, raw->rpb_table, (const long long*)raw->rpb_index,
                 (float*)at(pl.bqkv), (float*)at(pl.w9), (float*)at(pl.w9_flip), (float*)at(pl.dense), (float*)at(pl.tab), C, heads};
    const int n_small = 3 * C + 72 * C + heads * (4096 + 225);
    {
        BlockPackJobs j;
        j.m[0] = MatJob{raw->to_q_w, raw->to_kv_w, C, 3 * C, C, at(pl.wqkv), at(pl.wqkv_t), at(pl.wqkv_fm)};
        j.m[1] = MatJob{raw->proj_w, nullptr, C, C, C, at(pl.wp), at(pl.wp_t), at(pl.wp_fm)};
        j.m[2] = MatJob{raw->lin1_w, nullptr, 4 * C, 4 * C, C, at(pl.w1), at(pl.w1_t), at(pl.w1_fm)};
        j.m[3] = MatJob{raw->lin2_w, nullptr, C, C, 4 * C, at(pl.w2), at(pl.w2_t), at(pl.w2_fm)};
        int end = 0;
        for (int q = 0; q < 4; ++q) {
            end += (int)(((long long)j.m[q].N * (j.m[q].K / 8) + 255) / 256);
            j.e[q] = end;
        }
        j.sp = sp;
        j.n_small_blocks = (n_small + 255) / 256;
        UF_DISPATCH(dtype, TT, hipLaunchKernelGGL(pack_block_kernel<TT>, dim3((unsigned)(end + j.n_small_blocks)), dim3(256), 0, st, j));
    }
    if (int rc = check_launch("pack_block_train")) return rc;
    if (fwd) {
        *fwd = uf_block_params{};
        fwd->norm1_w = raw->norm1_w; fwd->norm1_b = raw->norm1_b; fwd->modulator = raw->modulator;
        fwd->rpb_dense = (const float*)at(pl.dense); fwd->rpb_fm = nullptr; fwd->rpb_tab = raw->index_is_standard ? (const float*)at(pl.tab) : nullptr;
        fwd->wqkv_fm = at(pl.wqkv_fm); fwd->bqkv = (const float*)at(pl.bqkv);
        fwd->wproj = at(pl.wp); fwd->wproj_fm = at(pl.wp_fm); fwd->bproj = raw->proj_b;
        fwd->norm2_w = raw->norm2_w; fwd->norm2_b = raw->norm2_b;
        fwd->w1_fm = at(pl.w1_fm); fwd->b1 = raw->lin1_b; fwd->wdw9 = (const float*)at(pl.w9); fwd->bdw = raw->dw_b;
        fwd->w2_fm = at(pl.w2_fm); fwd->b2 = raw->lin2_b;
        fwd->shift = shift; fwd->heads = heads;
    }
    if (bwd) {
        *bwd = uf_block_train_params{};
        bwd->norm1_w = raw->norm1_w; bwd->norm1_b = raw->norm1_b; bwd->norm2_w = raw->norm2_w; bwd->norm2_b = raw->norm2_b;
        bwd->modulator = raw->modulator; bwd->rpb_dense = (const float*)at(pl.dense);
        bwd->wqkv = at(pl.wqkv); bwd->wqkv_t = at(pl.wqkv_t); bwd->bqkv = (const float*)at(pl.bqkv);
        bwd->wproj = at(pl.wp); bwd->wproj_t = at(pl.wp_t); bwd->bproj = raw->proj_b;
        bwd->w1 = at(pl.w1); bwd->w1_t = at(pl.w1_t); bwd->b1 = raw->lin1_b;
        bwd->wdw9 = (const float*)at(pl.w9); bwd->wdw9_flip = (const float*)at(pl.w9_flip); bwd->bdw = raw->dw_b;
        bwd->w2_t = at(pl.w2_t); bwd->w2 = at(pl.w2);
        bwd->shift = shift; bwd->heads = heads;
    }
    return UF_OK;
}
```

### uformer_amd/model.py

```python
from __future__ import annotations

from typing import Optional, Tuple

import torch
import torch.nn as nn

from . import _lib, ops, packing
from ._lib import UformerHipError
from .spec import MAX_IN_CHANS, STAGES, UformerConfig, check_image_chans, relative_position_index
from .train import block_hw

Tensor = torch.Tensor
HW = Optional[Tuple[int, int]]


def window_partition(x: Tensor, win_size: int, dilation_rate: int = 1) -> Tensor:
    if dilation_rate != 1:
        raise NotImplementedError("dilation_rate != 1 is never exercised by the reference (SURVEY.md section 2 row 1)")
    return ops.window_partition(x, win_size, 0)


def window_reverse(windows: Tensor, win_size: int, H: int, W: int, dilation_rate: int = 1) -> Tensor:
    if dilation_rate != 1:
        raise NotImplementedError("dilation_rate != 1 is never exercised by the reference")
# ... 220 lines not shown
        self.out_features = out_features

    def forward(self, x: Tensor, compute_dtype=torch.float32, *, hw: HW = None) -> Tensor:
        bs, L, c = x.shape
        a = _to_compute(x.reshape(bs * L, c), compute_dtype)
        h = ops.linear(a, _to_compute(self.fc1.weight, compute_dtype), self.fc1.bias.detach().float(), 1)
        y = ops.linear(h, _to_compute(self.fc2.weight, compute_dtype), self.fc2.bias.detach().float(), 0)
        return y.reshape(bs, L, self.out_features).to(x.dtype)

    def flops(self, H, W):
        return H * W * self.in_features * self.hidden_features + H * W * self.hidden_features * self.out_features


class Downsample(nn.Module):

    def __init__(self, in_channel, out_channel):
        super().__init__()
        self.conv = nn.Sequential(nn.Conv2d(in_channel, out_channel, kernel_size=4, stride=2, padding=1))
        self.in_channel = in_channel
        self.out_channel = out_channel

    def forward(self, x: Tensor, compute_dtype=torch.float32, *, hw: HW = None) -> Tensor:
        B, L, Cc = x.shape
        H, W = block_hw(L, hw, "Downsample")
        y = ops.downsample(x.reshape(B * L, Cc), packing.pack_downsample(self.conv[0].weight, compute_dtype),
                           self.conv[0].bias.detach().float(), B, H, W)
        return y.reshape(B, L // 4, self.out_channel)

    def flops(self, H, W):
        return H / 2 * W / 2 * self.in_channel * self.out_channel * 4 * 4


class Upsample(nn.Module):

    def __init__(self, in_channel, out_channel):
        super().__init__()
        self.deconv = nn.Sequential(nn.ConvTranspose2d(in_channel, out_channel, kernel_size=2, stride=2))
        self.in_channel = in_channel
        self.out_channel = out_channel

    def forward(self, x: Tensor, compute_dtype=torch.float32, *, hw: HW = None) -> Tensor:
        B, L, Cc = x.shape
        H, W = block_hw(L, hw, "Upsample")
        y = ops.upsample(x.reshape(B * L, Cc), packing.pack_upsample(self.deconv[0].weight, compute_dtype),
                         self.deconv[0].bias.detach().float(), B, H, W)
        return y.reshape(B, 4 * L, self.out_channel)

    def flops(self, H, W):
        return H * W * self.in_channel * self.out_channel


class InputProj(nn.Module):

    def __init__(self, in_channel=3, out_channel=64, kernel_size=3, stride=1, norm_layer=None, act_layer=nn.LeakyReLU):
        super().__init__()
        if norm_layer is not None or kernel_size != 3 or stride != 1 or act_layer is not nn.LeakyReLU:
            raise NotImplementedError("InputProj: only the configuration Uformer builds (model.py:1100)")
        if in_channel < 1:
            raise NotImplementedError(f"InputProj: in_channel={in_channel}")
        self.proj = nn.Sequential(nn.Conv2d(in_channel, out_channel, kernel_size=3, stride=stride, padding=kernel_size // 2),
                                  act_layer(inplace=True))
        self.in_channel = in_channel
        self.out_channel = out_channel

    def forward(self, x: Tensor) -> Tensor:
        B, Cc, H, W = x.shape
        y = ops.input_proj(x, packing.pack_input_proj(self.proj[0].weight), self.proj[0].bias.detach().float())
        return y.reshape(B, H * W, self.out_channel)

    def flops(self, H, W):
        return H * W * self.in_channel * self.out_channel * 9


class OutputProj(nn.Module):

    def __init__(self, in_channel=64, out_channel=3, kernel_size=3, stride=1, norm_layer=None, act_layer=None):
        super().__init__()
        if norm_layer is not None or act_layer is not None or kernel_size != 3 or stride != 1 or not 1 <= out_channel <= MAX_IN_CHANS:
            raise NotImplementedError(f"OutputProj: only the configuration Uformer builds (model.py:1101), out_channel 1..{MAX_IN_CHANS}")
        self.proj = nn.Sequential(nn.Conv2d(in_channel, out_channel, kernel_size=3, stride=stride, padding=kernel_size // 2))
        self.in_channel = in_channel
        self.out_channel = out_channel

    def forward(self, x: Tensor, img: Optional[Tensor] = None, *, hw: HW = None) -> Tensor:
        B, L, Cc = x.shape
        H, W = block_hw(L, hw if hw is not None or img is None else tuple(img.shape[-2:]), "OutputProj")
        return ops.output_proj(x.reshape(B * L, Cc), packing.pack_output_proj(self.proj[0].weight),
                               self.proj[0].bias.detach().float(), B, H, W, img)

    def flops(self, H, W):
        return H * W * self.in_channel * self.out_channel * 9


class LeWinTransformerBlock(nn.Module):

    def __init__(self, dim, input_resolution, num_heads, win_size=8, shift_size=0, mlp_ratio=4., qkv_bias=True,
                 qk_scale=None, drop=0., attn_drop=0., drop_path=0., act_layer=nn.GELU, norm_layer=nn.LayerNorm,
                 token_projection='linear', token_mlp='leff', modulator=False, cross_modulator=False):
        super().__init__()
        if token_mlp not in ('leff', 'ffn', 'mlp'):
            raise NotImplementedError(f"token_mlp={token_mlp!r}: 'leff' and 'ffn' / 'mlp' are built ('fastleff' needs a third-party CUDA package, "
                                      "model.py:895-896)")
        if norm_layer is not nn.LayerNorm or drop:
            raise NotImplementedError("LayerNorm / drop=0 only")
        self.dim = dim
        self.input_resolution = tuple(input_resolution)
        self.num_heads = num_heads
        self.win_size = win_size
        self.shift_size = shift_size
        self.mlp_ratio = mlp_ratio
        self.token_mlp = token_mlp
        self.token_projection = token_projection
        if min(self.input_resolution) <= self.win_size:
            self.shift_size = 0
            self.win_size = min(self.input_resolution)
        assert 0 <= self.shift_size < self.win_size, "shift_size must in 0-win_size"
        if win_size != 8 or self.win_size not in (4, 8):
            raise NotImplementedError(f"the HIP path is built for win_size 8 and for a window clamped to 4; this block would need window "
                                      f"{self.win_size} (input_resolution {tuple(self.input_resolution)}, win_size {win_size})")
        if self.win_size == 4 and modulator:
            raise NotImplementedError("a 4x4-window block with a modulator: the reference's (64, C) embedding (model.py:868-869) does not broadcast "
                                      "onto 16-token windows (model.py:967-969)")
        self.modulator = nn.Embedding(win_size * win_size, dim) if modulator else None
        if cross_modulator:
            if self.win_size != 8:
                raise NotImplementedError("cross_modulator is built for 8x8-window blocks (img_size 64 clamps the bottleneck's window to 4)")
            self.cross_modulator = nn.Embedding(win_size * win_size, dim)
            self.cross_attn = Attention(dim, num_heads, qkv_bias=qkv_bias, qk_scale=qk_scale, attn_drop=attn_drop, proj_drop=drop,
                                        token_projection=token_projection)
            self.norm_cross = norm_layer(dim)
        else:
            self.cross_modulator = None
        self.norm1 = norm_layer(dim)
        self.attn = WindowAttention(dim, win_size=(self.win_size, self.win_size), num_heads=num_heads, qkv_bias=qkv_bias,
                                    qk_scale=qk_scale, attn_drop=attn_drop, proj_drop=drop, token_projection=token_projection)
        self.drop_path_rate = float(drop_path)
        self.norm2 = norm_layer(dim)
        if token_mlp == 'leff':
            self.mlp = LeFF(dim, int(dim * mlp_ratio), act_layer=act_layer, drop=drop)
        else:
            if self.win_size == 4 or dim > 512 or dim not in (16, 32, 64, 128, 256, 512):
                raise NotImplementedError(f"token_mlp={token_mlp!r} is built for 8x8-window blocks of width 16 ... 512 (uf_ffn_fwd); this block has "
                                          f"width {dim} and window {self.win_size} (img_size 64 and embed_dim 64 take token_mlp='leff' only)")
            self.mlp = Mlp(in_features=dim, hidden_features=int(dim * mlp_ratio), act_layer=act_layer, drop=drop)
        self._packed = None
        self._packed_cross = None

    def extra_repr(self) -> str:
        return (f"dim={self.dim}, input_resolution={self.input_resolution}, num_heads={self.num_heads}, "
                f"win_size={self.win_size}, shift_size={self.shift_size}, mlp_ratio={self.mlp_ratio}")

    def _pack(self, dtype):
        sd = {k: v for k, v in self.state_dict(keep_vars=True).items()}
        key = (dtype, tuple((v.data_ptr(), v._version) for v in sd.values()))
        if self._packed is None or self._packed[0] != key:
            if self.win_size == 4:
                bp, keep = packing.pack_block4(sd, "", self.num_heads, dtype)
            else:
                bp, keep = packing.pack_block(sd, "", self.num_heads, self.shift_size, dtype)
            self._packed = (key, bp, keep)
        return self._packed[1]

    def _pack_cross(self, dtype):
        sd = {k: v for k, v in self.state_dict(keep_vars=True).items() if k.startswith(("cross_modulator.", "cross_attn."))}
        key = (dtype, tuple((v.data_ptr(), v._version) for v in sd.values()))
        if self._packed_cross is None or self._packed_cross[0] != key:
            cp, keep = packing.pack_cross(sd, "", self.num_heads, dtype)
            self._packed_cross = (key, cp, keep)
        return self._packed_cross[1]
# ... 250 lines not shown
        if self.cfg.stage_windows()[4] == 4 and x.dim() == 4:
            for name, n in (("H", x.shape[2]), ("W", x.shape[3])):
                if n % 64 or n <= 0:
                    raise UformerHipError(f"{name}={n} must be a positive multiple of 64 (a model built for img_size {self.reso}: "
                                          f"4 downsamplings x the bottleneck's 4x4 windows)")
            if mask is not None:
                raise NotImplementedError("the mask argument is not supported by a model whose bottleneck runs on 4x4 windows (img_size 64; "
                                          "no reference script passes it)")
        if not x.is_cuda:
            raise UformerHipError("uformer_amd.Uformer runs on an MI355X only; there is no CPU fallback "
                                  "(the CPU oracle lives in oracle/ and is test infrastructure)")
        if x.dim() != 4 or x.shape[1] != self.dd_in:
            raise UformerHipError(f"expected (B,{self.dd_in},H,W) input, got {tuple(x.shape)}")
        if torch.is_grad_enabled() and (self.training or x.requires_grad or any(p.requires_grad for p in self.parameters())):
            if mask is None:
                return self._forward_train(x)
            if self.training or x.requires_grad:
                raise NotImplementedError("the mask argument is not supported by the autograd path (no reference script passes it): "
                                          "wrap the call in torch.no_grad() for inference")
            if not getattr(self, "_warned_eval_mask", False):
                import warnings
                warnings.warn("uformer_amd.Uformer: eval() forward with a mask while grad mode is on runs the inference kernels; the result has no "
                              "grad_fn (wrap the call in torch.no_grad() to silence this)", stacklevel=2)
                self._warned_eval_mask = True
        if mask is not None:
            return self._forward_blockwise(x, mask)
        B, _, H, W = x.shape
        xin = x.detach().float().contiguous()
        dt = ops.uf_dtype(self.compute_dtype)
        with torch.cuda.device(x.device):
            lib = _lib.load()
            pk = self._get_packed(x.device)
            if pk.win4:
                need = lib.uf_uformer_win4_workspace_bytes(pk.desc, B, H, W, dt)
                if need == 0:
                    raise UformerHipError("uf_uformer_win4_workspace_bytes: " + _lib.last_error())
                ws = self._workspace(need, x.device)
                out = torch.empty((B, self.in_chans, H, W), dtype=torch.float32, device=x.device)
                _lib.check(lib.uf_uformer_win4_fwd(pk.desc, pk.bneck, xin.data_ptr(), out.data_ptr(), B, H, W, dt, ws.data_ptr(),
                                                   ws.numel(), torch.cuda.current_stream().cuda_stream), "uf_uformer_win4_fwd")
                return out.to(x.dtype)
            need = lib.uf_uformer_workspace_bytes(pk.desc, B, H, W, dt)
            if need == 0:
                raise UformerHipError("uf_uformer_workspace_bytes: " + _lib.last_error())
            ws = self._workspace(need, x.device)
            out = torch.empty((B, self.in_chans, H, W), dtype=torch.float32, device=x.device)
            _lib.check(lib.uf_uformer_fwd(pk.desc, xin.data_ptr(), out.data_ptr(), B, H, W, dt, ws.data_ptr(),
                                          ws.numel(), torch.cuda.current_stream().cuda_stream), "uf_uformer_fwd")
        return out.to(x.dtype)

    def drop_path_rates(self):
        from .spec import STAGES
        return [float(blk.drop_path_rate) for name in STAGES for blk in getattr(self, name).blocks]

    def _forward_train(self, x: Tensor) -> Tensor:
        from . import train
        self._check_not_replica()
        sd = self.state_dict(keep_vars=True)
        names, params = list(sd.keys()), list(sd.values())
        sink = getattr(self, "grad_sink", None)
        names = train.NamesWithSink(names)
        names.sink = sink
        names.recompute = True if (self.use_checkpoint and self.compute_dtype in (torch.bfloat16, torch.float16)) else None
        rates = self.drop_path_rates() if self.training else []
        drop = getattr(self, "_drop_scales_override", None) if self.training else None
        if drop is None and any(r > 0 for r in rates):
            drop = train.sample_drop_scales(rates, x.shape[0], x.device)
        return train.UformerFunction.apply(x, self.cfg, self.compute_dtype, drop, names, *params)

    def _forward_blockwise(self, x: Tensor, mask: Optional[Tensor]) -> Tensor:
        cd = self.compute_dtype
        H, W = x.shape[-2:]
        r = [(H // d, W // d) for d in (1, 2, 4, 8, 16)]
        y = self.input_proj(x.detach().float())
        conv0 = self.encoderlayer_0(y, mask, cd, hw=r[0])
        conv1 = self.encoderlayer_1(self.dowsample_0(conv0, cd, hw=r[0]), mask, cd, hw=r[1])
        conv2 = self.encoderlayer_2(self.dowsample_1(conv1, cd, hw=r[1]), mask, cd, hw=r[2])
        conv3 = self.encoderlayer_3(self.dowsample_2(conv2, cd, hw=r[2]), mask, cd, hw=r[3])
        conv4 = self.conv(self.dowsample_3(conv3, cd, hw=r[3]), mask, cd, hw=r[4])
        d0 = self.decoderlayer_0(torch.cat([self.upsample_0(conv4, cd, hw=r[4]), conv3], -1), mask, cd, hw=r[3])
        d1 = self.decoderlayer_1(torch.cat([self.upsample_1(d0, cd, hw=r[3]), conv2], -1), mask, cd, hw=r[2])
        d2 = self.decoderlayer_2(torch.cat([self.upsample_2(d1, cd, hw=r[2]), conv1], -1), mask, cd, hw=r[1])
        d3 = self.decoderlayer_3(torch.cat([self.upsample_3(d2, cd, hw=r[1]), conv0], -1), mask, cd, hw=r[0])
        out = self.output_proj(d3, x.detach().float() if self.dd_in == 3 else None, hw=r[0])
        return out.to(x.dtype)

    def flops(self):
        total = 0
        r = self.reso
        total += self.input_proj.flops(r, r) + self.output_proj.flops(r, r)
        dims = self.cfg.stage_dims()
        div = self.cfg.stage_res_div()
        wins = self.cfg.stage_windows()
        for s in range(9):
            L = (r // div[s]) ** 2
            total += self.cfg.depths[s] * L * dims[s] * (12 * dims[s] + 2 * wins[s] ** 2 + (0 if self.cfg.mlp_is_ffn() else 36)
                                                         + (27 if self.cfg.token_projection == 'conv' else 0))
            if self.cfg.stage_has_cross_modulator(s):
                total += self.cfg.depths[s] * (2 * L * dims[s] * dims[s] + 2 * 64 * dims[s] * dims[s] + 2 * L * dims[s] * 64)
        for s in range(4):
            L = (r // div[s]) ** 2
            total += (L // 4) * dims[s] * 2 * dims[s] * 16
        for k, (cin, cout) in enumerate(self.cfg.upsample_io()):
            L = (r // div[4 + k]) ** 2
            total += 4 * L * cin * cout
        return total


class ConvBlock(nn.Module):

    def __init__(self, in_channel, out_channel, strides=1):
        super().__init__()
        if strides != 1:
            raise NotImplementedError(f"ConvBlock(strides={strides}): the HIP UNet runs stride-1 blocks only (the reference's UNet uses no other)")
        self.strides = strides
        self.in_channel = in_channel
        self.out_channel = out_channel
        self.block = nn.Sequential(
            nn.Conv2d(in_channel, out_channel, kernel_size=3, stride=strides, padding=1),
            nn.LeakyReLU(inplace=True),
            nn.Conv2d(out_channel, out_channel, kernel_size=3, stride=strides, padding=1),
            nn.LeakyReLU(inplace=True),
        )
        self.conv11 = nn.Conv2d(in_channel, out_channel, kernel_size=1, stride=strides, padding=0)

    def flops(self, H, W):
        return H * W * self.in_channel * self.out_channel * (3 * 3 + 1) + H * W * self.out_channel * self.out_channel * 3 * 3


class UNet(nn.Module):

    def __init__(self, block=ConvBlock, dim=32, compute_dtype=torch.bfloat16):
        super().__init__()
        if compute_dtype not in (torch.float32, torch.bfloat16, torch.float16):
            raise ValueError(f"compute_dtype must be float32, bfloat16 or float16, got {compute_dtype}")
        if dim not in (16, 32, 64, 128):
            raise ValueError(f"UNet(dim={dim}): dim must be 16, 32, 64 or 128 (conv10 runs on the OutputProj kernel, which takes those widths)")
        self.dim = dim
        self.compute_dtype = compute_dtype
        self.ConvBlock1 = ConvBlock(3, dim, strides=1)
        self.pool1 = nn.Conv2d(dim, dim, kernel_size=4, stride=2, padding=1)
        self.ConvBlock2 = block(dim, dim * 2, strides=1)
        self.pool2 = nn.Conv2d(dim * 2, dim * 2, kernel_size=4, stride=2, padding=1)
        self.ConvBlock3 = block(dim * 2, dim * 4, strides=1)
        self.pool3 = nn.Conv2d(dim * 4, dim * 4, kernel_size=4, stride=2, padding=1)
        self.ConvBlock4 = block(dim * 4, dim * 8, strides=1)
        self.pool4 = nn.Conv2d(dim * 8, dim * 8, kernel_size=4, stride=2, padding=1)
        self.ConvBlock5 = block(dim * 8, dim * 16, strides=1)
        self.upv6 = nn.ConvTranspose2d(dim * 16, dim * 8, 2, stride=2)
        self.ConvBlock6 = block(dim * 16, dim * 8, strides=1)
        self.upv7 = nn.ConvTranspose2d(dim * 8, dim * 4, 2, stride=2)
        self.ConvBlock7 = block(dim * 8, dim * 4, strides=1)
        self.upv8 = nn.ConvTranspose2d(dim * 4, dim * 2, 2, stride=2)
        self.ConvBlock8 = block(dim * 4, dim * 2, strides=1)
        self.upv9 = nn.ConvTranspose2d(dim * 2, dim, 2, stride=2)
        self.ConvBlock9 = block(dim * 2, dim, strides=1)
        self.conv10 = nn.Conv2d(dim, 3, kernel_size=3, stride=1, padding=1)
        self._packed = None
        self._ws = None

    MAX_WORKSPACES = Uformer.MAX_WORKSPACES
    _workspace = Uformer._workspace

    def _apply(self, fn, *a, **k):
        self._packed = None
        self._ws = None
        return super()._apply(fn, *a, **k)
# ... 92 lines not shown
```

### uformer_amd/ops.py

```python
from __future__ import annotations

from typing import Optional

import torch

from . import _lib
from ._lib import UF_BF16, UF_F16, UF_F32, UformerHipError

Tensor = torch.Tensor


def uf_dtype(dtype) -> int:
    if dtype in (UF_F32, UF_BF16, UF_F16) and not isinstance(dtype, torch.dtype):
        return int(dtype)
    if dtype == torch.float32:
        return UF_F32
    if dtype == torch.bfloat16:
        return UF_BF16
    if dtype == torch.float16:
        return UF_F16
    raise UformerHipError(f"unsupported operand dtype {dtype} (torch.float32, torch.bfloat16 or torch.float16)")


def torch_dtype(dt: int) -> torch.dtype:
# ... 554 lines not shown


def lewin_attn_train_fwd(bp, x: Tensor, B: int, H: int, W: int, heads: int, dtype, drop_attn: Optional[Tensor] = None):
    _dev(x, drop_attn)
    x = _c(x, torch.float32)
    M, Cc = x.shape
    T, hd = torch_dtype(uf_dtype(dtype)), Cc // heads
    dev = x.device
    x1 = torch.empty_like(x)
    xn, o, z = (torch.empty((M, Cc), dtype=T, device=dev) for _ in range(3))
    q = torch.empty((M // 64, heads, 64, hd), dtype=T, device=dev)
    k = torch.empty_like(q)
    vt = torch.empty((M // 64, heads, hd, 64), dtype=T, device=dev)
    a1 = torch.empty((M, 4 * Cc), dtype=T, device=dev)
    da = None if drop_attn is None else _c(drop_attn, torch.float32)
    with torch.cuda.device(dev):
        _lib.check(_lib.load().uf_lewin_attn_train_fwd(bp, _ptr(x), Cc, _ptr(x1), Cc, B, H, W, Cc, _ptr(da), uf_dtype(dtype), _ptr(xn), _ptr(q), _ptr(k), _ptr(vt),
                                                       _ptr(o), _ptr(z), _ptr(a1), _stream()), "uf_lewin_attn_train_fwd")
    return x1, xn, q, k, vt, o, z, a1


def pack_weight_fm(w: Tensor) -> Tensor:
    return _pack_frag(w)


def downsample(x: Tensor, w_packed: Tensor, bias: Tensor, B: int, H: int, W: int, w_fm: Optional[Tensor] = None) -> Tensor:
    _dev(x, w_packed, bias)
    x = _c(x, torch.float32)
    Cc = x.shape[-1]
    out = torch.empty((B * (H // 2) * (W // 2), 2 * Cc), dtype=torch.float32, device=x.device)
    with torch.cuda.device(x.device):
        if w_fm is not None:
            _lib.check(_lib.load().uf_downsample_fm_fwd(_ptr(x), Cc, _ptr(_c(w_packed)), _ptr(_c(w_fm)), _ptr(_c(bias, torch.float32)), _ptr(out),
                                                        2 * Cc, B, H, W, Cc, uf_dtype(w_packed.dtype), _stream()), "uf_downsample_fm_fwd")
        else:
            _lib.check(_lib.load().uf_downsample_fwd(_ptr(x), Cc, _ptr(_c(w_packed)), _ptr(_c(bias, torch.float32)), _ptr(out),
                                                     2 * Cc, B, H, W, Cc, uf_dtype(w_packed.dtype), _stream()), "uf_downsample_fwd")
    return out


def upsample(x: Tensor, w_packed: Tensor, bias: Tensor, B: int, H: int, W: int, out: Optional[Tensor] = None,
             ld_o: Optional[int] = None) -> Tensor:
    _dev(x, w_packed, bias)
    x = _c(x, torch.float32)
    Cin = x.shape[-1]
    Cout = w_packed.shape[0] // 4
    if out is None:
        out = torch.empty((B * 4 * H * W, Cout), dtype=torch.float32, device=x.device)
        ld_o = Cout
    with torch.cuda.device(x.device):
        _lib.check(_lib.load().uf_upsample_fwd(_ptr(x), Cin, _ptr(_c(w_packed)), _ptr(_c(bias, torch.float32)), _ptr(out), ld_o,
                                               B, H, W, Cin, Cout, uf_dtype(w_packed.dtype), _stream()), "uf_upsample_fwd")
    return out


def input_proj(img: Tensor, w27: Tensor, bias: Tensor) -> Tensor:
    _dev(img, w27, bias)
    img = _c(img, torch.float32)
    B, Cin, H, W = img.shape
    E = w27.shape[1]
    out = torch.empty((B * H * W, E), dtype=torch.float32, device=img.device)
    with torch.cuda.device(img.device):
        _lib.check(_lib.load().uf_input_proj_fwd(_ptr(img), _ptr(_c(w27, torch.float32)), _ptr(_c(bias, torch.float32)),
                                                 _ptr(out), E, B, Cin, H, W, E, _stream()), "uf_input_proj_fwd")
    return out


def output_proj(x: Tensor, w: Tensor, bias: Tensor, B: int, H: int, W: int, img: Optional[Tensor] = None) -> Tensor:
    _dev(x, w, bias, img)
    x = _c(x, torch.float32)
    C2 = x.shape[-1]
    Cout = w.shape[0]
    if w.dim() != 3 or tuple(w.shape[1:]) != (9, C2) or bias.numel() != Cout:
        raise UformerHipError(f"output_proj: w {tuple(w.shape)} / bias {tuple(bias.shape)} do not match (Cout, 9, {C2}) / (Cout,)")
    if img is not None:
        img = _c(img, torch.float32)
        if tuple(img.shape) != (B, Cout, H, W):
            raise UformerHipError(f"output_proj: img {tuple(img.shape)} must have the output's shape {(B, Cout, H, W)}")
    out = torch.empty((B, Cout, H, W), dtype=torch.float32, device=x.device)
    with torch.cuda.device(x.device):
        _lib.check(_lib.load().uf_output_proj_c_fwd(_ptr(x), C2, _ptr(_c(w, torch.float32)), _ptr(_c(bias, torch.float32)),
                                                    _ptr(img), _ptr(out), B, H, W, C2, Cout, int(img is not None), _stream()),
                   "uf_output_proj_c_fwd")
    return out


def _byref(struct):
    import ctypes
    return ctypes.byref(struct)


def _ws(nbytes: int, device) -> Tensor:
    return torch.empty(max(int(nbytes), 16), dtype=torch.uint8, device=device)


def charbonnier(y: Tensor, target: Tensor, eps: float = 1e-3, with_grad: bool = True, grad_scale: float = 1.0):
    _dev(y, target)
    y, target = _c(y, torch.float32), _c(target, torch.float32)
    n = y.numel()
    loss = torch.empty(1, dtype=torch.float32, device=y.device)
    dy = torch.empty_like(y) if with_grad else None
    lib = _lib.load()
    nbytes = lib.uf_charbonnier_workspace_bytes(n)
    ws = _ws(nbytes, y.device)
    with torch.cuda.device(y.device):
        _lib.check(lib.uf_charbonnier_fwd_bwd(_ptr(y), _ptr(target), _ptr(dy), _ptr(loss), n, eps, grad_scale, _ptr(ws), nbytes, _stream()),
                   "uf_charbonnier_fwd_bwd")
    return loss.reshape(()), dy


def adamw_step(params, grads, exp_avg, exp_avg_sq, *, lr: float, betas=(0.9, 0.999), eps: float = 1e-8, weight_decay: float = 0.02,
               step: int = 1, grad_scale: float = 1.0) -> None:
    import ctypes as C
    n = len(params)
    if not (len(grads) == len(exp_avg) == len(exp_avg_sq) == n):
        raise UformerHipError("adamw_step: list lengths differ")
    if n == 0:
        return
    dev = _dev(*params, *grads, *exp_avg, *exp_avg_sq)
    for group in (params, grads, exp_avg, exp_avg_sq):
        for t in group:
            if t.dtype != torch.float32 or not t.is_contiguous():
                raise UformerHipError("adamw_step: tensors must be contiguous float32")
    arr = lambda ts: (C.c_void_p * n)(*[t.data_ptr() for t in ts])
    numel = (C.c_longlong * n)(*[p.numel() for p in params])
    with torch.cuda.device(dev):
        _lib.check(_lib.load().uf_adamw_step(arr(params), arr(grads), arr(exp_avg), arr(exp_avg_sq), numel, n, lr, betas[0], betas[1], eps,
                                             weight_decay, int(step), grad_scale, _stream()), "uf_adamw_step")


def adamw_step_scaled(params, grads, exp_avg, exp_avg_sq, scaler_state: Tensor, *, lr: float, betas=(0.9, 0.999), eps: float = 1e-8, weight_decay: float = 0.02,
                      grad_scale: float = 1.0) -> None:
    import ctypes as C
    n = len(params)
    if not (len(grads) == len(exp_avg) == len(exp_avg_sq) == n):
        raise UformerHipError("adamw_step_scaled: list lengths differ")
    if n == 0:
        return
    dev = _dev(*params, *grads, *exp_avg, *exp_avg_sq, scaler_state)
    for group in (params, grads, exp_avg, exp_avg_sq, [scaler_state]):
        for t in group:
            if t.dtype != torch.float32 or not t.is_contiguous():
                raise UformerHipError("adamw_step_scaled: tensors must be contiguous float32")
    arr = lambda ts: (C.c_void_p * n)(*[t.data_ptr() for t in ts])
    numel = (C.c_longlong * n)(*[p.numel() for p in params])
    with torch.cuda.device(dev):
        _lib.check(_lib.load().uf_adamw_step_scaled(arr(params), arr(grads), arr(exp_avg), arr(exp_avg_sq), numel, n, lr, betas[0], betas[1], eps,
                                                    weight_decay, grad_scale, _ptr(scaler_state), _stream()), "uf_adamw_step_scaled")


def grad_scaler_check(grads, scaler_state: Tensor) -> None:
    import ctypes as C
    grads = [g for g in grads if g is not None]
    n = len(grads)
    if n == 0:
        return
    dev = _dev(*grads, scaler_state)
    for t in grads:
        if t.dtype != torch.float32 or not t.is_contiguous():
            raise UformerHipError("grad_scaler_check: gradients must be contiguous float32")
    arr = (C.c_void_p * n)(*[t.data_ptr() for t in grads])
    numel = (C.c_longlong * n)(*[t.numel() for t in grads])
    with torch.cuda.device(dev):
        _lib.check(_lib.load().uf_grad_scaler_check(arr, numel, n, _ptr(scaler_state), _stream()), "uf_grad_scaler_check")


# ... 327 lines not shown
```

### uformer_amd/packing.py

```python
from __future__ import annotations

import ctypes as C
from typing import Dict, List

import torch

from . import _lib

Tensor = torch.Tensor


def rpb_dense(table: Tensor, index: Tensor) -> Tensor:
    n = index.shape[0]
    return table.detach()[index.reshape(-1)].reshape(n, n, -1).permute(2, 0, 1).contiguous().float()


def pack_frag(w: Tensor, dtype: torch.dtype) -> Tensor:
    N, K = w.shape
    KP = (K + 31) // 32 * 32
    w = w.detach().to(dtype)
    if KP != K:
        w = torch.nn.functional.pad(w, (0, KP - K))
    return w.reshape(N // 16, 16, KP // 32, 4, 8).permute(0, 2, 3, 1, 4).contiguous()


def pack_rpb_table(dense: Tensor):
    h = dense.shape[0]
    c = torch.arange(8, device=dense.device)
    ys, xs = torch.meshgrid(c, c, indexing="ij")
    ys, xs = ys.reshape(-1), xs.reshape(-1)
    row = (ys[:, None] - ys[None, :] + 7)
    pos = (7 - (xs[:, None] - xs[None, :]))
    tab = torch.zeros(h, 15, 15, dtype=torch.float32, device=dense.device)
    tab[:, row, pos] = dense.float()
    if not torch.equal(tab[:, row, pos], dense.float()):
        return None
    return tab.contiguous()


def pack_rpb_table4(table: Tensor, index: Tensor) -> Tensor:
    dense = rpb_dense(table, index)
    if dense.shape[1:] != (16, 16):
        raise ValueError(f"pack_rpb_table4: expected a (16, 16) relative_position_index, got {tuple(index.shape)}")
    c = torch.arange(4, device=dense.device)
    ys, xs = torch.meshgrid(c, c, indexing="ij")
    ys, xs = ys.reshape(-1), xs.reshape(-1)
    ent = (ys[:, None] - ys[None, :] + 3) * 7 + (xs[:, None] - xs[None, :] + 3)
    tab = torch.zeros(dense.shape[0], 49, dtype=torch.float32, device=dense.device)
    tab[:, ent] = dense
    if not torch.equal(tab[:, ent], dense):
        raise ValueError("pack_rpb_table4: the relative-position bias is not Toeplitz in (dy, dx); the 4x4-window kernels need the "
                         "reference's relative_position_index")
    return tab.contiguous()


def pack_dwconv(w: Tensor) -> Tensor:
    return w.detach().reshape(w.shape[0], 9).t().contiguous().float()


def conv_projection_keys(sd: Dict[str, Tensor], prefix: str) -> bool:
    return (prefix + "attn.qkv.to_q.depthwise.weight") in sd


def pack_conv_projection(sd: Dict[str, Tensor], prefix: str):
    g = lambda j, k: sd[prefix + f"attn.qkv.to_{j}.{k}"].detach()
    wpw = torch.cat([g(j, "pointwise.weight").reshape(g(j, "pointwise.weight").shape[0], -1) for j in "qkv"], 0)
    bpw = torch.cat([g(j, "pointwise.bias") for j in "qkv"], 0).contiguous().float()
    dw9 = torch.stack([pack_dwconv(g(j, "depthwise.weight")) for j in "qkv"], 0).contiguous()
    bdw = torch.stack([g(j, "depthwise.bias").float() for j in "qkv"], 0).contiguous()
    return wpw, bpw, dw9, bdw


def pack_downsample(w: Tensor, dtype: torch.dtype) -> Tensor:
    return w.detach().permute(0, 2, 3, 1).reshape(w.shape[0], -1).contiguous().to(dtype)


def pack_upsample(w: Tensor, dtype: torch.dtype) -> Tensor:
    return w.detach().permute(2, 3, 1, 0).reshape(-1, w.shape[0]).contiguous().to(dtype)


def pack_input_proj(w: Tensor) -> Tensor:
    return w.detach().permute(1, 2, 3, 0).reshape(-1, w.shape[0]).contiguous().float()


def pack_output_proj(w: Tensor) -> Tensor:
    return w.detach().permute(0, 2, 3, 1).reshape(w.shape[0], 9, w.shape[1]).contiguous().float()


def pack_block(sd: Dict[str, Tensor], prefix: str, heads: int, shift: int, dtype: torch.dtype):
    f = lambda k: sd[prefix + k].detach().float().clone().contiguous()
    t = lambda k: sd[prefix + k].detach().to(dtype, copy=True).contiguous()
    conv = conv_projection_keys(sd, prefix)
    if conv:
        wqkv, bqkv, dw9, bdw = pack_conv_projection(sd, prefix)
    else:
        wqkv = torch.cat([sd[prefix + "attn.qkv.to_q.weight"].detach(), sd[prefix + "attn.qkv.to_kv.weight"].detach()], 0)
        bqkv = torch.cat([sd[prefix + "attn.qkv.to_q.bias"].detach(), sd[prefix + "attn.qkv.to_kv.bias"].detach()], 0).contiguous().float()
    dense = rpb_dense(sd[prefix + "attn.relative_position_bias_table"], sd[prefix + "attn.relative_position_index"])
    keep: Dict[str, Tensor] = {
        "norm1_w": f("norm1.weight"), "norm1_b": f("norm1.bias"),
        "rpb_dense": dense,
        "wqkv_fm": pack_frag(wqkv, dtype),
        "bqkv": bqkv,
        "wproj": t("attn.proj.weight"), "wproj_fm": pack_frag(sd[prefix + "attn.proj.weight"], dtype), "bproj": f("attn.proj.bias"),
        "norm2_w": f("norm2.weight"), "norm2_b": f("norm2.bias"),
    }
    if (prefix + "mlp.fc1.weight") in sd:
        keep.update({"w1_fm": pack_frag(sd[prefix + "mlp.fc1.weight"], dtype), "b1": f("mlp.fc1.bias"),
                     "w2_fm": pack_frag(sd[prefix + "mlp.fc2.weight"], dtype), "b2": f("mlp.fc2.bias")})
    else:
        keep.update({"w1_fm": pack_frag(sd[prefix + "mlp.linear1.0.weight"], dtype), "b1": f("mlp.linear1.0.bias"),
                     "wdw9": pack_dwconv(sd[prefix + "mlp.dwconv.0.weight"]), "bdw": f("mlp.dwconv.0.bias"),
                     "w2_fm": pack_frag(sd[prefix + "mlp.linear2.0.weight"], dtype), "b2": f("mlp.linear2.0.bias")})
    if conv:
        keep.update({"qkv_dw9": dw9, "qkv_bdw": bdw})
    if (prefix + "modulator.weight") in sd:
        keep["modulator"] = f("modulator.weight")
    tab = pack_rpb_table(dense)
    if tab is not None:
        keep["rpb_tab"] = tab
    bp = _lib.BlockParams()
    for name, _ in _lib.BlockParams._fields_:
        if name in ("shift", "heads"):
            continue
        setattr(bp, name, keep[name].data_ptr() if name in keep else None)
    bp.shift = int(shift)
    bp.heads = int(heads)
    return bp, keep


def cross_modulator_keys(sd: Dict[str, Tensor], prefix: str) -> bool:
    return (prefix + "cross_modulator.weight") in sd


def pack_cross(sd: Dict[str, Tensor], prefix: str, heads: int, dtype: torch.dtype):
    cp = _lib.CrossParams()
    if not cross_modulator_keys(sd, prefix):
        return cp, {}
    g = lambda k: sd[prefix + k].detach()
    emb = g("cross_modulator.weight").float()
    n, C = emb.shape
    if n != 64 or C % heads or C // heads not in (16, 32):
        raise NotImplementedError(f"cross_modulator: built for 64 learned tokens and head_dim 16 or 32 (uf_cross_attn_fwd); this block has {n} tokens, "
                                  f"width {C} and {heads} heads")
    hd = C // heads
    kv = torch.nn.functional.linear(emb, g("cross_attn.qkv.to_kv.weight").float(), g("cross_attn.qkv.to_kv.bias").float())
    keep: Dict[str, Tensor] = {
        "wq_fm": pack_frag(g("cross_attn.qkv.to_q.weight"), dtype),
        "bq": g("cross_attn.qkv.to_q.bias").float().clone().contiguous(),
        "k": kv[:, :C].reshape(64, heads, hd).permute(1, 0, 2).to(dtype).contiguous(),
        "vt": kv[:, C:].reshape(64, heads, hd).permute(1, 2, 0).to(dtype).contiguous(),
        "wp_fm": pack_frag(g("cross_attn.proj.weight"), dtype),
        "bp": g("cross_attn.proj.bias").float().clone().contiguous(),
    }
    for name, tns in keep.items():
        setattr(cp, name, tns.data_ptr())
    cp.heads = int(heads)
    return cp, keep


def pack_block4(sd: Dict[str, Tensor], prefix: str, heads: int, dtype: torch.dtype):
    if cross_modulator_keys(sd, prefix):
        raise NotImplementedError("cross_modulator is not built for 4x4-window blocks (the bottleneck of an img_size-64 model)")
    """``uf_block4_params`` of a 4x4-window block (row-major T weights, the (heads, 49) bias table): returns (Block4Params, keepalive)."""
    if conv_projection_keys(sd, prefix):
        raise NotImplementedError("token_projection='conv' is not built for 4x4-window blocks (the bottleneck of an img_size-64 model)")
    if (prefix + "mlp.fc1.weight") in sd:
        raise NotImplementedError("token_mlp='ffn' is not built for 4x4-window blocks (the bottleneck of an img_size-64 model)")
    if (prefix + "modulator.weight") in sd:
# ... 124 lines not shown
```

Baseline: 2513.

## Fuse output-projection channel contraction into last LeFF epilogue, add tap-sum kernel

The output 3x3 conv is split into two steps. A per-pixel contraction of the C channels into 27 tap partials (z) is done with fp32 MFMA inside the epilogue of the last decoder block's LeFF kernel. A small tiled kernel then sums the nine shifted taps, adds bias and image, and writes the output. This avoids re-reading the full C-channel activation for the head conv, at the cost of disabling the persistent schedule for that LeFF launch and writing a 32-wide float z buffer.

```diff
diff --git a/include/uformer_hip.h b/include/uformer_hip.h
--- a/include/uformer_hip.h
+++ b/include/uformer_hip.h
@@ -142,6 +142,13 @@
 int uf_output_proj_c_fwd(const float* x, int ld_x, const float* w, const float* bias,
                          const float* img, float* out, int B, int H, int W, int C2, int Cout, int add_img,
                          void* stream);
+
+int uf_pack_head_wz(const float* w, float* wz, int C, int Cout, void* stream);
+int uf_head_z_fwd(const float* x, int ld_x, const float* wz, float* z, long long M, int C, void* stream);
+int uf_leff_head_z_fwd(const uf_block_params* p, const float* x, int ld, const float* wz, float* z, int B, int H, int W, int C,
+                       uf_dtype dtype, void* ws, size_t ws_bytes, void* stream);
+int uf_head_taps_fwd(const float* z, const float* bias, const float* img, float* out, int B, int H, int W, int Cout, int add_img,
+                     void* stream);
 
 int uf_gelu_bwd(const void* a, const void* dy, void* dx, long long n, uf_dtype dtype, void* stream);
 int uf_gelu_fwd(const void* a, void* y, long long n, uf_dtype dtype, void* stream);
diff --git a/uformer_amd/_lib.py b/uformer_amd/_lib.py
--- a/uformer_amd/_lib.py
+++ b/uformer_amd/_lib.py
@@ -130,6 +130,10 @@
     "uf_input_proj_fwd": (I, [P, P, P, P, I, I, I, I, I, I, P]),
     "uf_output_proj_fwd": (I, [P, I, P, P, P, P, I, I, I, I, I, P]),
     "uf_output_proj_c_fwd": (I, [P, I, P, P, P, P, I, I, I, I, I, I, P]),
+    "uf_pack_head_wz": (I, [P, P, I, I, P]),
+    "uf_head_z_fwd": (I, [P, I, P, P, C.c_longlong, I, P]),
+    "uf_leff_head_z_fwd": (I, [C.POINTER(BlockParams), P, I, P, P, I, I, I, I, I, P, c_size_t, P]),
+    "uf_head_taps_fwd": (I, [P, P, P, P, I, I, I, I, I, P]),
     "uf_rows_sum_workspace_bytes": (c_size_t, [I, I]),
     "uf_rows_sum": (I, [P, I, P, I, I, I, P, c_size_t, P]),
     "uf_rpb_table_grad": (I, [P, P, I, P]),
diff --git a/uformer_amd/csrc/uf_elementwise.hip b/uformer_amd/csrc/uf_elementwise.hip
--- a/uformer_amd/csrc/uf_elementwise.hip
+++ b/uformer_amd/csrc/uf_elementwise.hip
@@ -1,4 +1,7 @@
+#include <limits.h>
+
 #include "uf_internal.h"
+#include "uf_headtaps.h"
 
 namespace uf {
 namespace {
@@ -829,3 +832,121 @@
                                   int B, int H, int W, int C2, int add_img, void* stream) {
     return uf_output_proj_c_fwd(x, ld_x, w, bias, img, out, B, H, W, C2, 3, add_img, stream);
 }
+
+namespace uf {
+namespace {
+
+template <int C>
+__global__ __launch_bounds__(256) void head_z_kernel(const float* __restrict__ x, int ld_x, const float* __restrict__ wz, float* __restrict__ z, long long M) {
+    constexpr int NT = C / 16;
+    const int lane = threadIdx.x & 63, fr = lane & 15, fg = lane >> 4;
+    const long long row0 = ((long long)blockIdx.x * 4 + (threadIdx.x >> 6)) * 16;
+    if (row0 >= M) return;
+    const long long row = row0 + fr, rr = row < M ? row : M - 1;
+    const float* xr = x + (size_t)rr * ld_x + fg * 4;
+    f32x4 q0[NT], q1[NT];
+#pragma unroll
+    for (int i = 0; i < NT; ++i) {
+        const f32x4 xv = *reinterpret_cast<const f32x4*>(xr + 16 * i);
+        q0[i] = head_z_tile(head_wz_load(wz, i, 0, lane), xv);
+        q1[i] = head_z_tile(head_wz_load(wz, i, 1, lane), xv);
+    }
+    const f32x4 s0 = head_z_tree<NT>(q0), s1 = head_z_tree<NT>(q1);
+    if (row < M) {
+        float* zp = z + (size_t)row * HZ_W + fg * 4;
+        *reinterpret_cast<f32x4*>(zp) = s0;
+        *reinterpret_cast<f32x4*>(zp + 16) = s1;
+    }
+}
+
+constexpr int HT_TH = 8, HT_TW = 32, HT_HW = HT_TW + 2;
+template <int CO>
+__global__ __launch_bounds__(256) void head_taps_kernel(const float* __restrict__ z, const float* __restrict__ bias, const float* __restrict__ img,
+                                                        float* __restrict__ out, int B, int H, int W, int add_img, int tiles_x, int tiles_y) {
+    constexpr int NPART = (9 * CO + 3) / 4;
+    constexpr int HT_PS = NPART * 4 + 1;
+    constexpr int NPIECE = (HT_TH + 2) * HT_HW * 8, NIT = (NPIECE + 255) / 256;
+    __shared__ float tile[(HT_TH + 2) * HT_HW * HT_PS];
+    const int tid = threadIdx.x;
+    const int bt = xcd_tile(blockIdx.x, gridDim.x);
+    const int b = bt / (tiles_x * tiles_y), tr = bt - b * (tiles_x * tiles_y);
+    const int y0 = (tr / tiles_x) * HT_TH, x0 = (tr % tiles_x) * HT_TW;
+    f32x4 v[NIT];
+#pragma unroll
+    for (int k = 0; k < NIT; ++k) {
+        const int q = tid + k * 256, hp = q >> 3, part = q & 7;
+        const int hy = hp / HT_HW, hx = hp - hy * HT_HW;
+        const int iy = y0 - 1 + hy, ix = x0 - 1 + hx;
+        v[k] = f32x4{0.f, 0.f, 0.f, 0.f};
+        if (q < NPIECE && part < NPART && iy >= 0 && iy < H && ix >= 0 && ix < W) v[k] = *reinterpret_cast<const f32x4*>(z + (((size_t)b * H + iy) * W + ix) * HZ_W + part * 4);
+    }
+#pragma unroll
+    for (int k = 0; k < NIT; ++k) {
+        const int q = tid + k * 256, hp = q >> 3, part = q & 7;
+        if (q < NPIECE && part < NPART) {
+            float* d = tile + hp * HT_PS + part * 4;
+            d[0] = v[k][0]; d[1] = v[k][1]; d[2] = v[k][2]; d[3] = v[k][3];
+        }
+    }
+    __syncthreads();
+    const int ty = tid >> 5, tx = tid & 31, y = y0 + ty, xw = x0 + tx;
+    if (y >= H || xw >= W) return;
+    float acc[CO];
+#pragma unroll
+    for (int o = 0; o < CO; ++o) acc[o] = 0.f;
+#pragma unroll
+    for (int t = 0; t < 9; ++t) {
+        const int dy = t / 3 - 1, dx = t % 3 - 1;
+        if (y + dy >= 0 && y + dy < H && xw + dx >= 0 && xw + dx < W) {
+            const float* p = tile + ((ty + 1 + dy) * HT_HW + tx + 1 + dx) * HT_PS + t * CO;
+#pragma unroll
+            for (int o = 0; o < CO; ++o) acc[o] += p[o];
+        }
+    }
+#pragma unroll
+    for (int o = 0; o < CO; ++o) {
+        const size_t off = (((size_t)b * CO + o) * H + y) * W + xw;
+        float v = acc[o] + bias[o];
+        if (add_img) v += img[off];
+        out[off] = v;
+    }
+}
+
+}
+}
+
+extern "C" int uf_head_z_fwd(const float* x, int ld_x, const float* wz, float* z, long long M, int C, void* stream) {
+    UF_REQUIRE(x && wz && z, UF_ERR_NULL, "uf_head_z_fwd: null pointer");
+    UF_REQUIRE(C == 32 || C == 64 || C == 128, UF_ERR_UNSUPPORTED, "uf_head_z_fwd: C=%d unsupported (32,64,128)", C);
+    UF_REQUIRE(M > 0 && (M + 63) / 64 <= (long long)INT_MAX && ld_x >= C && ld_x % 4 == 0, UF_ERR_SHAPE, "uf_head_z_fwd: M=%lld ld_x=%d", M, ld_x);
+    UF_REQUIRE(((uintptr_t)x % 16) == 0 && ((uintptr_t)wz % 16) == 0 && ((uintptr_t)z % 16) == 0, UF_ERR_ALIGN, "uf_head_z_fwd: operands must be 16-byte aligned");
+    hipStream_t st = (hipStream_t)stream;
+    {
+        ScopedTimer tm("head_z", 2.0 * M * C * HZ_W, 4.0 * M * (C + HZ_W), st);
+        const dim3 grid((unsigned)((M + 63) / 64));
+        if (C == 32) hipLaunchKernelGGL(head_z_kernel<32>, grid, dim3(256), 0, st, x, ld_x, wz, z, M);
+        else if (C == 64) hipLaunchKernelGGL(head_z_kernel<64>, grid, dim3(256), 0, st, x, ld_x, wz, z, M);
+        else hipLaunchKernelGGL(head_z_kernel<128>, grid, dim3(256), 0, st, x, ld_x, wz, z, M);
+    }
+    return check_launch("head_z");
+}
+
+extern "C" int uf_head_taps_fwd(const float* z, const float* bias, const float* img, float* out, int B, int H, int W, int Cout, int add_img,
+                                void* stream) {
+    UF_REQUIRE(z && bias && out && (!add_img || img), UF_ERR_NULL, "uf_head_taps_fwd: null pointer");
+    UF_REQUIRE(Cout >= 1 && 9 * Cout <= HZ_W, UF_ERR_UNSUPPORTED, "uf_head_taps_fwd: Cout=%d unsupported (1..3: nine taps per plane in a %d-wide row)", Cout, HZ_W);
+    UF_REQUIRE(B > 0 && H > 0 && W > 0, UF_ERR_SHAPE, "uf_head_taps_fwd: B=%d H=%d W=%d", B, H, W);
+    UF_REQUIRE(((uintptr_t)z % 16) == 0, UF_ERR_ALIGN, "uf_head_taps_fwd: z must be 16-byte aligned");
+    hipStream_t st = (hipStream_t)stream;
+    const int tiles_x = (W + HT_TW - 1) / HT_TW, tiles_y = (H + HT_TH - 1) / HT_TH;
+    const long long nt = (long long)tiles_x * tiles_y * B, pix = (long long)B * H * W;
+    UF_REQUIRE(nt <= (long long)INT_MAX, UF_ERR_SHAPE, "uf_head_taps_fwd: too many tiles (pixels are indexed in 64 bits: the grid is the limit)");
+    {
+        ScopedTimer tm("head_taps", 10.0 * Cout * pix, 4.0 * pix * (HZ_W + (add_img ? 2 : 1) * Cout), st);
+        const dim3 grid((unsigned)nt);
+        if (Cout == 1) hipLaunchKernelGGL(head_taps_kernel<1>, grid, dim3(256), 0, st, z, bias, img, out, B, H, W, add_img, tiles_x, tiles_y);
+        else if (Cout == 2) hipLaunchKernelGGL(head_taps_kernel<2>, grid, dim3(256), 0, st, z, bias, img, out, B, H, W, add_img, tiles_x, tiles_y);
+        else hipLaunchKernelGGL(head_taps_kernel<3>, grid, dim3(256), 0, st, z, bias, img, out, B, H, W, add_img, tiles_x, tiles_y);
+    }
+    return check_launch("head_taps");
+}
diff --git a/uformer_amd/csrc/uf_headtaps.h b/uformer_amd/csrc/uf_headtaps.h
--- /dev/null
+++ b/uformer_amd/csrc/uf_headtaps.h
@@ -0,0 +1,30 @@
+#pragma once
+#include "uf_common.h"
+
+namespace uf {
+
+constexpr int HZ_W = 32;
+
+__device__ __forceinline__ f32x4 head_wz_load(const float* __restrict__ wz, int tile, int ot, int lane) {
+    return *reinterpret_cast<const f32x4*>(wz + ((size_t)(tile * 2 + ot) * 64 + lane) * 4);
+}
+
+__device__ __forceinline__ f32x4 head_z_tile(const f32x4 wa, const f32x4 x) {
+    f32x4 d = f32x4{0.f, 0.f, 0.f, 0.f};
+    d = __builtin_amdgcn_mfma_f32_16x16x4f32(wa[0], x[0], d, 0, 0, 0);
+    d = __builtin_amdgcn_mfma_f32_16x16x4f32(wa[1], x[1], d, 0, 0, 0);
+    d = __builtin_amdgcn_mfma_f32_16x16x4f32(wa[2], x[2], d, 0, 0, 0);
+    d = __builtin_amdgcn_mfma_f32_16x16x4f32(wa[3], x[3], d, 0, 0, 0);
+    return d;
+}
+
+template <int N> __device__ __forceinline__ f32x4 head_z_tree(f32x4 (&p)[N]) {
+    static_assert((N & (N - 1)) == 0, "power of two");
+#pragma unroll
+    for (int s = 1; s < N; s *= 2)
+#pragma unroll
+        for (int i = 0; i < N; i += 2 * s) p[i] = p[i] + p[i + s];
+    return p[0];
+}
+
+}
diff --git a/uformer_amd/csrc/uf_internal.h b/uformer_amd/csrc/uf_internal.h
--- a/uformer_amd/csrc/uf_internal.h
+++ b/uformer_amd/csrc/uf_internal.h
@@ -47,7 +47,7 @@
 int launch_attn_block(const uf_block_params* bp, float* x, int ld, int B, int H, int W, int C, uf_dtype dtype, void* h1_out, hipStream_t st,
                       const float* drop = nullptr, float* xo = nullptr, int ldo = 0);
 int launch_leff2(const void* h1, const float* w9, const float* bdw, const void* W2, const float* b2, float* x, int ld, int B, int H, int W, int C,
-                 uf_dtype dtype, const float* drop, hipStream_t st);
+                 uf_dtype dtype, const float* drop, hipStream_t st, const float* wz = nullptr, float* z = nullptr);
 
 int launch_attn_block_train(const uf_block_params* bp, const float* x, int ld, float* x1, int ld1, int B, int H, int W, int C, uf_dtype dtype, const float* drop,
                             void* xn, void* q, void* k, void* vt, void* o, void* z, void* a1, hipStream_t st);
diff --git a/uformer_amd/csrc/uf_leff2.hip b/uformer_amd/csrc/uf_leff2.hip
--- a/uformer_amd/csrc/uf_leff2.hip
+++ b/uformer_amd/csrc/uf_leff2.hip
@@ -2,6 +2,7 @@
 
 #include "uf_internal.h"
 #include "uf_mconv.h"
+#include "uf_headtaps.h"
 
 namespace uf {
 namespace {
@@ -15,6 +16,7 @@
     int B, H, W;
     int n_tiles;
     unsigned long long* tbuf;
+    const float* wz; float* z;
 };
 
 constexpr int KCW = 64;
@@ -33,7 +35,7 @@
     *reinterpret_cast<f32x4*>(p + 4) = f32x4{f[4], f[5], f[6], f[7]};
 }
 
-template <typename T, int C, int NPG, int NC, int NBUF, int WPS, int PW = 4, int CP = 0>
+template <typename T, int C, int NPG, int NC, int NBUF, int WPS, int PW = 4, int CP = 0, int ZT = 0>
 __global__ __launch_bounds__((PW * NPG + NC) * 64, WPS) void leff2_kernel(const Leff2Params p) {
     constexpr int NP = PW * NPG;
     constexpr int MC = sizeof(T) == 2 ? 1 : 0;
@@ -63,6 +65,7 @@
     constexpr int AT_BYTES = BM * SAT;
     constexpr int WN = (C / 16) < NC ? (C / 16) : NC, WM = NC / WN;
     static_assert(WM <= 4, "consumer grid");
+    static_assert(ZT == 0 || (sizeof(T) == 2 && CP == 0 && NC == 4 && C >= 32 && C <= 128), "head-taps epilogue: 2-byte operands, four consumer waves = four pixel tiles");
     constexpr int TMW = 4 / WM, TNW = (C / 16) / WN;
     extern __shared__ __attribute__((aligned(16))) char smem[];
     char* Ring = smem;
@@ -282,7 +285,34 @@
                 else if (j < NTOT) w2_issue(0);
                 __builtin_amdgcn_sched_barrier(0);
             }
-            if (it == NIT - 1) {
+            if (it == NIT - 1 && ZT != 0) {
+                static_assert(ZT == 0 || WN * 4 * 2 * 64 * 16 <= NBUF * BUFB, "z partials fit the DMA ring");
+                const float dscale = p.drop ? p.drop[tb] : 1.0f;
+#pragma unroll
+                for (int i = 0; i < TNW; ++i) {
+                    const f32x4 b2 = *reinterpret_cast<const f32x4*>(p.b2 + (wn * TNW + i) * 16 + fg * 4);
+#pragma unroll
+                    for (int jj = 0; jj < TMW; ++jj) {
+                        f32x4 r;
+                        if constexpr (XPRE) r = xres[i][jj]; else r = *reinterpret_cast<const f32x4*>(x_ptr(tb, ty0, tx0, i, jj));
+                        acc[i][jj] = r + (acc[i][jj] + b2) * dscale;
+                    }
+                }
+#pragma unroll
+                for (int ot = 0; ot < 2; ++ot) {
+                    f32x4 wa[TNW];
+#pragma unroll
+                    for (int i = 0; i < TNW; ++i) wa[i] = *reinterpret_cast<const f32x4*>(reinterpret_cast<const char*>(p.wz) + ((wn * TNW + i) * 2 + ot) * 1024 + wlane);
+#pragma unroll
+                    for (int jj = 0; jj < TMW; ++jj) {
+                        f32x4 q[TNW];
+#pragma unroll
+                        for (int i = 0; i < TNW; ++i) q[i] = head_z_tile(wa[i], acc[i][jj]);
+                        *reinterpret_cast<f32x4*>(Ring + ((wn * 4 + wm * TMW + jj) * 2 + ot) * 1024 + wlane) = head_z_tree<TNW>(q);
+                    }
+                    __builtin_amdgcn_sched_barrier(0);
+                }
+            } else if (it == NIT - 1) {
                 const float dscale = p.drop ? p.drop[tb] : 1.0f;
 #pragma unroll
                 for (int i = 0; i < TNW; ++i) {
@@ -309,6 +339,19 @@
         lds_barrier();
         ct1 = __builtin_readcyclecounter(); ctbar += ct1 - ct0; ct0 = ct1;
     }
+    if constexpr (ZT != 0) {
+        int tb, ty0, tx0;
+        tile_coords(0, tb, ty0, tx0);
+        const int pm = cw * 16 + fr;
+        float* zp = p.z + ((size_t)(tb * p.H + ty0 + (pm >> 3)) * p.W + tx0 + (pm & 7)) * HZ_W + fg * 4;
+#pragma unroll
+        for (int ot = 0; ot < 2; ++ot) {
+            f32x4 part[WN];
+#pragma unroll
+            for (int w = 0; w < WN; ++w) part[w] = *reinterpret_cast<const f32x4*>(Ring + ((w * 4 + cw) * 2 + ot) * 1024 + wlane);
+            *reinterpret_cast<f32x4*>(zp + ot * 16) = head_z_tree<WN>(part);
+        }
+    }
     if (p.tbuf && lane == 0 && (bt & 63) == 0) { p.tbuf[((bt >> 6) * 16 + wave) * 4] = ctw; p.tbuf[((bt >> 6) * 16 + wave) * 4 + 1] = ctbar; p.tbuf[((bt >> 6) * 16 + wave) * 4 + 2] = 0; }
     if (cw == 0 && lane == 0) {
         Census c2 = census;
@@ -317,23 +360,24 @@
     }
 }
 
-template <typename T, int C, int NPG, int NC, int NBUF, int WPS, int PW = 4, int CP = 0>
+template <typename T, int C, int NPG, int NC, int NBUF, int WPS, int PW = 4, int CP = 0, int ZT = 0>
 int launch_v(const Leff2Params& p, hipStream_t st) {
     constexpr int SZ = sizeof(T), KC = KCW * NPG;
     constexpr int HGB = (100 * KCW * SZ + 1023) / 1024 * 1024, TGB = (10 * KC * 4 + 1023) / 1024 * 1024;
     constexpr int smem = NBUF * (NPG * HGB + TGB) + 2 * 64 * (KC * SZ + 16) + 1024;
     static_assert(smem <= 160 * 1024, "LDS budget");
-    auto kern = leff2_kernel<T, C, NPG, NC, NBUF, WPS, PW, CP>;
+    auto kern = leff2_kernel<T, C, NPG, NC, NBUF, WPS, PW, CP, ZT>;
     static bool lds_done[64] = {};
     if (int rc = ensure_dynamic_lds(reinterpret_cast<const void*>(kern), smem, lds_done, "leff2")) return rc;
     const long long M = (long long)p.B * p.H * p.W;
     char name[96] = "";
-    if (timing_enabled()) snprintf(name, sizeof(name), "leff2_%s_c%d_np%d_nc%d %lldx%dx%d", TypeName<T>::s, C, PW * NPG, NC, M, C, 4 * C);
+    if (timing_enabled()) snprintf(name, sizeof(name), "leff2%s_%s_c%d_np%d_nc%d %lldx%dx%d", ZT ? "z" : "", TypeName<T>::s, C, PW * NPG, NC, M, C, 4 * C);
     {
-        ScopedTimer tm(name, 2.0 * M * C * 4 * C + 18.0 * M * 4 * C, (double)M * 4 * C * SZ + (double)M * C * 8, st);
+        ScopedTimer tm(name, 2.0 * M * C * 4 * C + 18.0 * M * 4 * C + (ZT ? 2.0 * M * C * HZ_W : 0.0),
+                       (double)M * 4 * C * SZ + (double)M * C * 4 + (double)M * 4 * (ZT ? HZ_W : C), st);
         const int pe = variant("persist", -1);
         const bool pays = C <= 32 || C >= 256 || (C == 128 && p.n_tiles <= 1024);
-        const bool persist = pe >= 0 ? pe != 0 : pays;
+        const bool persist = ZT ? false : (pe >= 0 ? pe != 0 : pays);
         constexpr int waves = PW * NPG + NC;
         constexpr int by_lds = (160 * 1024) / smem, by_waves = 32 / waves, by_regs = (WPS * 4) / waves > 0 ? (WPS * 4) / waves : 1;
         constexpr int per_cu = by_lds < by_waves ? (by_lds < by_regs ? by_lds : by_regs) : (by_waves < by_regs ? by_waves : by_regs);
@@ -355,6 +399,12 @@
     if constexpr (sizeof(T) == 2 && C >= 32) {
         const int ev = variant("leff2", 0);
         const bool force = ev == 1, never = ev == 2;
+        if constexpr (C <= 128) {
+            if (p.z) {
+                const bool wide = C == 128 ? (!never && (force || tiles <= 1024)) : force;
+                return wide ? launch_v<T, C, 1, 4, 2, 6, 8, 0, 1>(p, st) : launch_v<T, C, 1, 4, 2, 6, 4, 0, 1>(p, st);
+            }
+        }
         if constexpr (C == 128) { if (!never && (force || tiles <= 1024)) return launch_v<T, C, 1, 4, 2, 6, 8>(p, st); }
         else if constexpr (C == 256) { if (!never && (force || tiles <= 256)) return launch_v<T, C, 1, 8, NB256E, 4, 8>(p, st); }
         else if constexpr (C == 512) { if (force) return launch_v<T, C, 1, 8, 4, 4, 8>(p, st); }
@@ -394,7 +444,7 @@
 
 namespace uf {
 int launch_leff2(const void* h1, const float* w9, const float* bdw, const void* W2, const float* b2, float* x, int ld, int B, int H, int W, int C,
-                 uf_dtype dtype, const float* drop, hipStream_t st) {
+                 uf_dtype dtype, const float* drop, hipStream_t st, const float* wz, float* z) {
     UF_REQUIRE(h1 && w9 && bdw && W2 && b2 && x, UF_ERR_NULL, "uf_dwconv_linear2_fwd: null pointer");
     UF_REQUIRE(B > 0 && H >= 8 && W >= 8 && H % 8 == 0 && W % 8 == 0, UF_ERR_SHAPE, "uf_dwconv_linear2_fwd: B=%d H=%d W=%d (multiples of 8)", B, H, W);
     UF_REQUIRE(ld >= C && ld % 4 == 0, UF_ERR_ALIGN, "uf_dwconv_linear2_fwd: ld=%d", ld);
@@ -404,7 +454,11 @@
     UF_REQUIRE((long long)H * W * 4LL * C * (long long)dtype_size(dtype) < 0xffffff00LL, UF_ERR_SHAPE,
                "uf_dwconv_linear2_fwd: one image of the hidden tensor must stay under 4 GiB (32-bit buffer offsets)");
     UF_REQUIRE((long long)B * H * W < 0x7fffffffLL / 4, UF_ERR_SHAPE, "uf_dwconv_linear2_fwd: too many tokens");
+    UF_REQUIRE(!wz == !z, UF_ERR_NULL, "uf_dwconv_linear2_fwd: the head weight pack and the z rows go together");
+    UF_REQUIRE(!z || (dtype_half(dtype) && (C == 32 || C == 64 || C == 128) && ((uintptr_t)wz % 16) == 0 && ((uintptr_t)z % 16) == 0), UF_ERR_UNSUPPORTED,
+               "leff2 head-taps epilogue: bf16 / f16 operands, C in {32, 64, 128}, 16-byte aligned operands (got dtype %d, C=%d)", (int)dtype, C);
     Leff2Params p{};
+    p.wz = wz; p.z = z;
     p.tbuf = debug_get_tbuf();
     p.h1 = h1; p.w9 = w9; p.bdw = bdw; p.W2 = W2; p.b2 = b2; p.x = x; p.ld = ld; p.B = B; p.H = H; p.W = W; p.drop = drop;
     p.n_tiles = B * (H / 8) * (W / 8);
diff --git a/uformer_amd/csrc/uf_model.hip b/uformer_amd/csrc/uf_model.hip
--- a/uformer_amd/csrc/uf_model.hip
+++ b/uformer_amd/csrc/uf_model.hip
@@ -122,9 +122,14 @@
     return uf_ffn_fwd(x, ld, p->norm2_w, p->norm2_b, p->w1_fm, p->b1, p->w2_fm, p->b2, drop, B, M, C, dtype, st);
 }
 
+bool head_taps_supported(const uf_block_params* p, uf_dtype dtype, int C, int in_chans) {
+    return dtype_half(dtype) && !mlp_block(p) && (C == 32 || C == 64 || C == 128) && in_chans >= 1 && in_chans <= 3;
+}
+
 int leff_half(const uf_block_params* p, float* x, int ld, int B, int H, int W, int C, uf_dtype dtype, const BlockWs& w,
-              hipStream_t st, bool fc1_done = false, const float* drop = nullptr) {
+              hipStream_t st, bool fc1_done = false, const float* drop = nullptr, const float* wz = nullptr, float* z = nullptr) {
     const int M = B * H * W;
+    UF_REQUIRE(!z || (!mlp_block(p) && !wide_block(C)), UF_ERR_UNSUPPORTED, "leff: the head-taps epilogue needs a LeFF block of C <= 128");
     if (mlp_block(p)) return mlp_half(p, x, ld, B, H, W, C, dtype, w, st, drop);
     if (wide_block(C)) {
         UF_REQUIRE(!drop && !fc1_done, UF_ERR_UNSUPPORTED, "leff: C=%d runs unfused, without DropPath scales", C);
@@ -148,7 +153,7 @@
         int rc = uf_ln_linear_gelu_fwd(x, ld, p->norm2_w, p->norm2_b, p->w1_fm, p->b1, w.h1, M, 4 * C, C, dtype, st);
         if (rc) return rc;
     }
-    return launch_leff2(w.h1, p->wdw9, p->bdw, p->w2_fm, p->b2, x, ld, B, H, W, C, dtype, drop, st);
+    return launch_leff2(w.h1, p->wdw9, p->bdw, p->w2_fm, p->b2, x, ld, B, H, W, C, dtype, drop, st, wz, z);
 }
 
 int block_fwd(const uf_block_params* p, float* x, int ld, int B, int H, int W, int C, const float* user_mask, int n_mask, uf_dtype dtype,
@@ -187,6 +192,19 @@
     rc = carve(w, ws, ws_bytes, (size_t)B * H * W, C, dtype);
     if (rc) return rc;
     return leff_half(p, x, ld, B, H, W, C, dtype, w, (hipStream_t)stream);
+}
+
+extern "C" int uf_leff_head_z_fwd(const uf_block_params* p, const float* x, int ld, const float* wz, float* z, int B, int H, int W, int C,
+                                 uf_dtype dtype, void* ws, size_t ws_bytes, void* stream) {
+    int rc = check_block_args(p, x, ld, B, H, W, C, dtype);
+    if (rc) return rc;
+    UF_REQUIRE(wz && z, UF_ERR_NULL, "uf_leff_head_z_fwd: null pointer");
+    UF_REQUIRE(head_taps_supported(p, dtype, C, 1), UF_ERR_UNSUPPORTED, "uf_leff_head_z_fwd: a LeFF block, bf16 / f16 operands, C in {32, 64, 128} (got dtype %d, C=%d)",
+               (int)dtype, C);
+    BlockWs w;
+    rc = carve(w, ws, ws_bytes, (size_t)B * H * W, C, dtype);
+    if (rc) return rc;
+    return leff_half(p, const_cast<float*>(x), ld, B, H, W, C, dtype, w, (hipStream_t)stream, false, nullptr, wz, z);
 }
 
 extern "C" int uf_mlp_fwd(const uf_block_params* p, float* x, int ld, int B, int H, int W, int C, uf_dtype dtype, void* ws,
@@ -358,12 +376,33 @@
         ld = 2 * pl.C[s];
     };
     const uf_block_params* blk = d->blocks;
+    int n_blocks = 0;
+    for (int s = 0; s < 9; ++s) n_blocks += d->depths[s];
+    const bool head_z = d->out_w && d->depths[8] > 0 && variant("headz", 1) != 0 && head_taps_supported(d->blocks + n_blocks - 1, dtype, pl.C[8], d->in_chans);
+    float* zrows = nullptr;
     auto run_stage = [&](int s, float* x, int ld) -> int {
         for (int i = 0; i < d->depths[s]; ++i, ++blk) {
             const uf_cross_params* cr = (d->cross && !bneck) ? d->cross + (blk - d->blocks) : nullptr;
             if (cr && cr->wq_fm) {
                 int r = uf_cross_attn_fwd(cr, x, ld, (int)pl.M[s], pl.C[s], dtype, st);
                 if (r) return r;
+            }
+            if (head_z && s == 8 && i == d->depths[8] - 1) {
+                int r = check_block_args(blk, x, ld, B, pl.res_h[s], pl.res_w[s], pl.C[s], dtype);
+                if (r) return r;
+                BlockWs w;
+                r = carve(w, bws, pl.blk_bytes, pl.M[s], pl.C[s], dtype);
+                if (r) return r;
+                bool fc1_done = false;
+                r = attn_half(blk, x, ld, B, pl.res_h[s], pl.res_w[s], pl.C[s], nullptr, 0, dtype, w, st, &fc1_done);
+                if (r) return r;
+                float* wz = reinterpret_cast<float*>(w.a);
+                r = uf_pack_head_wz(d->out_w, wz, pl.C[s], d->in_chans, st);
+                if (r) return r;
+                zrows = reinterpret_cast<float*>(w.h2);
+                r = leff_half(blk, x, ld, B, pl.res_h[s], pl.res_w[s], pl.C[s], dtype, w, st, fc1_done, nullptr, wz, zrows);
+                if (r) return r;
+                continue;
             }
             int r =(s == 4 && bneck) ? uf_lewin_block4_fwd(bneck + i, x, ld, B, pl.res_h[s], pl.res_w[s], pl.C[s], nullptr, nullptr, dtype, bws, pl.blk_bytes, st)
                                       : uf_lewin_block_fwd(blk, x, ld, B, pl.res_h[s], pl.res_w[s], pl.C[s], nullptr, 0, dtype, bws, pl.blk_bytes, st);
@@ -396,6 +435,7 @@
         rc = run_stage(s, x, ld);
         if (rc) return rc;
     }
+    if (zrows) return uf_head_taps_fwd(zrows, d->out_b, img, out, B, H, W, d->in_chans, d->dd_in == 3 ? 1 : 0, st);
     return uf_output_proj_c_fwd(x, ld, d->out_w, d->out_b, img, out, B, H, W, pl.C[8], d->in_chans, d->dd_in == 3 ? 1 : 0, st);
 }
 
diff --git a/uformer_amd/csrc/uf_pack.hip b/uformer_amd/csrc/uf_pack.hip
--- a/uformer_amd/csrc/uf_pack.hip
+++ b/uformer_amd/csrc/uf_pack.hip
@@ -155,3 +155,22 @@
     }
     return UF_OK;
 }
+
+namespace uf {
+namespace {
+__global__ void pack_head_wz_kernel(const float* __restrict__ w, float* __restrict__ wz, int C, int Cout) {
+    const int idx = blockIdx.x * blockDim.x + threadIdx.x;
+    if (idx >= C * 32) return;
+    const int r = idx & 3, lane = (idx >> 2) & 63, ot = (idx >> 8) & 1, i = idx >> 9;
+    const int fr = lane & 15, fg = lane >> 4, j = 16 * ot + fr, t = j / Cout, o = j - t * Cout;
+    wz[idx] = j < 9 * Cout ? w[(o * 9 + t) * C + 16 * i + 4 * fg + r] : 0.f;
+}
+}
+}
+
+extern "C" int uf_pack_head_wz(const float* w, float* wz, int C, int Cout, void* stream) {
+    UF_REQUIRE(w && wz, UF_ERR_NULL, "uf_pack_head_wz: null pointer");
+    UF_REQUIRE(C > 0 && C % 16 == 0 && Cout >= 1 && Cout <= 3, UF_ERR_UNSUPPORTED, "uf_pack_head_wz: C=%d (a multiple of 16), Cout=%d (1..3)", C, Cout);
+    hipLaunchKernelGGL(pack_head_wz_kernel, dim3((unsigned)(C * 32 + 255) / 256), dim3(256), 0, (hipStream_t)stream, w, wz, C, Cout);
+    return check_launch("pack_head_wz");
+}
diff --git a/uformer_amd/model.py b/uformer_amd/model.py
--- a/uformer_amd/model.py
+++ b/uformer_amd/model.py
@@ -326,9 +326,12 @@
         self.in_channel = in_channel
         self.out_channel = out_channel
 
-    def forward(self, x: Tensor, img: Optional[Tensor] = None, *, hw: HW = None) -> Tensor:
+    def forward(self, x: Tensor, img: Optional[Tensor] = None, *, hw: HW = None, compute_dtype: Optional[torch.dtype] = None) -> Tensor:
         B, L, Cc = x.shape
         H, W = block_hw(L, hw if hw is not None or img is None else tuple(img.shape[-2:]), "OutputProj")
+        if compute_dtype is not None and not self.training and packing.head_taps_supported(Cc, self.out_channel, compute_dtype):
+            z = ops.head_z(x.reshape(B * L, Cc), packing.pack_head_taps(self.proj[0].weight))
+            return ops.head_taps(z, self.proj[0].bias.detach().float(), B, H, W, img)
         return ops.output_proj(x.reshape(B * L, Cc), packing.pack_output_proj(self.proj[0].weight),
                                self.proj[0].bias.detach().float(), B, H, W, img)
 
@@ -745,7 +748,9 @@
         d1 = self.decoderlayer_1(torch.cat([self.upsample_1(d0, cd, hw=r[3]), conv2], -1), mask, cd, hw=r[2])
         d2 = self.decoderlayer_2(torch.cat([self.upsample_2(d1, cd, hw=r[2]), conv1], -1), mask, cd, hw=r[1])
         d3 = self.decoderlayer_3(torch.cat([self.upsample_3(d2, cd, hw=r[1]), conv0], -1), mask, cd, hw=r[0])
-        out = self.output_proj(d3, x.detach().float() if self.dd_in == 3 else None, hw=r[0])
+        last = self.decoderlayer_3.blocks
+        taps = len(last) > 0 and last[-1].token_mlp == 'leff'
+        out = self.output_proj(d3, x.detach().float() if self.dd_in == 3 else None, hw=r[0], compute_dtype=cd if taps else None)
         return out.to(x.dtype)
 
     def flops(self):
diff --git a/uformer_amd/ops.py b/uformer_amd/ops.py
--- a/uformer_amd/ops.py
+++ b/uformer_amd/ops.py
@@ -660,6 +660,34 @@
         _lib.check(_lib.load().uf_output_proj_c_fwd(_ptr(x), C2, _ptr(_c(w, torch.float32)), _ptr(_c(bias, torch.float32)),
                                                     _ptr(img), _ptr(out), B, H, W, C2, Cout, int(img is not None), _stream()),
                    "uf_output_proj_c_fwd")
+    return out
+
+
+def head_z(x: Tensor, wz: Tensor) -> Tensor:
+    _dev(x, wz)
+    x = _c(x, torch.float32)
+    M, C2 = x.shape
+    if wz.dtype != torch.float32 or wz.numel() != C2 * 32:
+        raise UformerHipError(f"head_z: wz {tuple(wz.shape)} {wz.dtype} does not match packing.pack_head_taps of a (Cout, {C2}, 3, 3) weight")
+    z = torch.empty((M, 32), dtype=torch.float32, device=x.device)
+    with torch.cuda.device(x.device):
+        _lib.check(_lib.load().uf_head_z_fwd(_ptr(x), C2, _ptr(_c(wz)), _ptr(z), M, C2, _stream()), "uf_head_z_fwd")
+    return z
+
+
+def head_taps(z: Tensor, bias: Tensor, B: int, H: int, W: int, img: Optional[Tensor] = None) -> Tensor:
+    _dev(z, bias, img)
+    Cout = bias.numel()
+    if z.dtype != torch.float32 or tuple(z.shape) != (B * H * W, 32) or not z.is_contiguous():
+        raise UformerHipError(f"head_taps: z {tuple(z.shape)} {z.dtype} must be contiguous float32 {(B * H * W, 32)}")
+    if img is not None:
+        img = _c(img, torch.float32)
+        if tuple(img.shape) != (B, Cout, H, W):
+            raise UformerHipError(f"head_taps: img {tuple(img.shape)} must have the output's shape {(B, Cout, H, W)}")
+    out = torch.empty((B, Cout, H, W), dtype=torch.float32, device=z.device)
+    with torch.cuda.device(z.device):
+        _lib.check(_lib.load().uf_head_taps_fwd(_ptr(z), _ptr(_c(bias, torch.float32)), _ptr(img), _ptr(out), B, H, W, Cout, int(img is not None),
+                                                _stream()), "uf_head_taps_fwd")
     return out
 
 
diff --git a/uformer_amd/packing.py b/uformer_amd/packing.py
--- a/uformer_amd/packing.py
+++ b/uformer_amd/packing.py
@@ -85,6 +85,26 @@
 
 def pack_output_proj(w: Tensor) -> Tensor:
     return w.detach().permute(0, 2, 3, 1).reshape(w.shape[0], 9, w.shape[1]).contiguous().float()
+
+
+HEAD_Z_WIDTH = 32
+HEAD_TAPS_WIDTHS = (32, 64, 128)
+
+
+def head_taps_supported(C2: int, cout: int, dtype) -> bool:
+    import os
+    if "headz=0" in os.environ.get("UF_VARIANT", "").split(","):
+        return False
+    return dtype in (torch.bfloat16, torch.float16) and C2 in HEAD_TAPS_WIDTHS and 1 <= cout <= 3
+
+
+def pack_head_taps(w: Tensor) -> Tensor:
+    co, c2 = w.shape[0], w.shape[1]
+    if co > 3 or c2 % 16:
+        raise ValueError(f"pack_head_taps: weight {tuple(w.shape)}: at most 3 planes, channels a multiple of 16")
+    wz = torch.zeros(HEAD_Z_WIDTH, c2, dtype=torch.float32, device=w.device)
+    wz[:9 * co] = w.detach().float().permute(2, 3, 0, 1).reshape(9 * co, c2)
+    return wz.reshape(2, 16, c2 // 16, 4, 4).permute(2, 0, 3, 1, 4).contiguous()
 
 
 def pack_block(sd: Dict[str, Tensor], prefix: str, heads: int, shift: int, dtype: torch.dtype):
```

Result: no change. 2540, median of 3 (+1.1%).
